# jzhangbs/MVSDF

Hardware: AMD Instinct MI355X
Metric: traced rays/sec (fwd+bwd, 10 sphere iters, 4 src views) (higher is better)
Workload: dtype f32x3

## Files before the change

include/mvsdf_hip.h:

```cpp
#ifndef MVSDF_HIP_H
#define MVSDF_HIP_H
#include <stddef.h>
#include <stdint.h>

#ifdef __cplusplus
extern "C" {
#endif

#define MVSDF_MAX_LAYERS 12

typedef struct {
    int n_layers;
    int K[MVSDF_MAX_LAYERS];
    int N[MVSDF_MAX_LAYERS];
    const float* wp[MVSDF_MAX_LAYERS];
    const float* bias[MVSDF_MAX_LAYERS];
    const float* w[MVSDF_MAX_LAYERS];
    int skip_layer;
    int multires;
    const void* wp16[MVSDF_MAX_LAYERS];
    int trace_dtype;
    unsigned skip_mask;
    const void* wx3[MVSDF_MAX_LAYERS];
} MvsdfNetDesc;

typedef struct {
    float r;
    float thr;
    float line_search_step;
    int line_step_iters;
    int st_iters;
    int n_steps;
    int n_secant;
    float dist_clip;
} MvsdfTraceParams;

enum {
    MVSDF_CNT_ROWS_SPHERE = 0,
    MVSDF_CNT_ROWS_SAMPLER = 1,
    MVSDF_CNT_ROWS_SECANT = 2,
    MVSDF_CNT_ROWS_MINSDF = 3,
    MVSDF_CNT_N_SECANT = 4,
    MVSDF_CNT_N_SAMPLER = 5,
    MVSDF_CNT_N_MINSDF = 6,
    MVSDF_CNT_N_SAMPLER_REST = 7,
    MVSDF_CNT_ROWS_SAMPLER_EVAL = 8,
    MVSDF_CNT_TAIL_NEXT = 9,
    MVSDF_CNT_TAIL_READY = 10,
    MVSDF_CNT_TAIL_WGS = 11,
    MVSDF_CNT_TAIL_ROWS = 12
};

int mvsdf_version(void);
int mvsdf_abi_struct_sizes(size_t* out);
const char* mvsdf_last_error(void);

size_t mvsdf_packed_floats(int N, int K);

int mvsdf_fold_pack(const float* v, const float* g, int N, int K, float* w, float* wp, float* wpT, void* stream);
int mvsdf_fold_pack_net(int n_layers, const float* const* v, const float* const* g, const int* N, const int* K, float* const* w,
                        float* const* wp, float* const* wpT, void* stream);
int mvsdf_fold_backward_net(int n_layers, const float* const* v, const float* const* g, const float* const* dW, const float* const* db,
                            const int* N, const int* K, float* const* dv, float* const* dg, float* const* dbias, int accumulate,
                            void* stream);
int mvsdf_fold_backward(const float* v, const float* g, const float* dW, int N, int K, float* dv, float* dg, void* stream);

size_t mvsdf_packed_bf16_bytes(int N, int K, int nsplit);
int mvsdf_pack_bf16w_net(int n_layers, const float* const* w, const int* N, const int* K, float* const* wp_rounded, void* stream);
int mvsdf_pack_bf16s_net(int n_layers, const float* const* w, const int* N, const int* K, void* const* wp16, void* stream);
int mvsdf_pack_bf16x3_net(int n_layers, const float* const* w, const int* N, const int* K, void* const* wp16, void* stream);
int mvsdf_pack_bf16x3t_net(int n_layers, const float* const* w, const int* N, const int* K, void* const* wx3t, void* stream);

int mvsdf_sdf_col0(const MvsdfNetDesc* net, const float* x, int n, float* y, int mt, void* stream);

int mvsdf_camera_rays(const float* uv, const float* pose, const float* intrinsics, int B, int P, float* ray_dirs, float* cam_loc,
                      void* stream);

int mvsdf_sphere_intersection(const float* cam_loc, const float* ray_dirs, int B, int P, float r, float* t, uint8_t* mask, void* stream);

size_t mvsdf_trace_workspace_bytes(int R);
size_t mvsdf_trace_workspace_bytes_n(int R, int n_steps);
int mvsdf_trace(const MvsdfNetDesc* net, const MvsdfTraceParams* tp, const float* cam_loc, const float* ray_dirs,
                const uint8_t* object_mask, int B, int P, int training, const float* intervals, const float* minsdf_steps,
                float* points, uint8_t* mask, float* dists, unsigned long long* counters, void* workspace,
                size_t workspace_bytes, int mt, int mt_samples, void* stream);
int mvsdf_trace_stage(int stage, const MvsdfNetDesc* net, const MvsdfTraceParams* tp, const float* cam_loc, const float* ray_dirs,
                      const uint8_t* object_mask, int B, int P, int training, const float* intervals, const float* minsdf_steps,
                      float* points, uint8_t* mask, float* dists, unsigned long long* counters, void* workspace,
                      size_t workspace_bytes, int mt, int mt_samples, void* stream);

size_t mvsdf_tracegen_state_bytes(int R);
int mvsdf_tracegen_init(const MvsdfTraceParams* tp, const float* cam_loc, const float* ray_dirs, const uint8_t* object_mask, int B, int P,
                        void* state, uint8_t* req, float* pts, unsigned long long* counters, void* stream);
int mvsdf_tracegen_step(const MvsdfTraceParams* tp, const float* cam_loc, const float* ray_dirs, int B, int P, void* state, const float* vals,
                        uint8_t* req, float* pts, unsigned long long* counters, void* stream);
int mvsdf_tracegen_finish(const MvsdfTraceParams* tp, const float* cam_loc, const float* ray_dirs, int B, int P, int training, const void* state,
                          float* points, uint8_t* mask, float* dists, unsigned long long* counters, void* workspace, size_t workspace_bytes,
                          void* stream);
int mvsdf_tracegen_rows(const MvsdfTraceParams* tp, int kind, const float* cam_loc, const float* ray_dirs, int B, int P, const float* zs, int n_list,
                        void* workspace, float* out_pts, void* stream);
int mvsdf_tracegen_reduce(const MvsdfTraceParams* tp, int kind, const float* cam_loc, const float* ray_dirs, int B, int P, int training,
                          const float* intervals, const float* minsdf_steps, const float* sv, float* points, uint8_t* mask, float* dists,
                          unsigned long long* counters, void* workspace, uint8_t* marks, void* stream);
int mvsdf_tracegen_secant(const MvsdfTraceParams* tp, int op, const float* cam_loc, const float* ray_dirs, int B, int P, int n_sec, const float* vals,
                          float* pts_out, float* points, float* dists, unsigned long long* counters, void* workspace, void* stream);

size_t mvsdf_sdf_ctx_floats(const MvsdfNetDesc* net, int M, int Mg);
int mvsdf_sdf_forward(const MvsdfNetDesc* net, const MvsdfNetDesc* netT, const float* x, int M, int Mg, float* y, float* nrm, float* ctx,
                      void* stream);
size_t mvsdf_sdf_bwd_ws_floats(const MvsdfNetDesc* net, int Mb);
int mvsdf_sdf_backward(const MvsdfNetDesc* net, const MvsdfNetDesc* netT, const float* x, int M, int Mg, int row0, int Mb, const float* dy,
                       const float* dn, const float* ctx, float* dW_cat, float* db_cat, float* dx, float* ws, void* stream);

int mvsdf_sdf_backward_pair(const MvsdfNetDesc* net, const MvsdfNetDesc* netT, int M, int Mg, int MbA, const float* dyA, const float* dnA, float* wsA,
                            int row0X, int MbX, const float* dyX, const float* dnX, float* wsX, float* dx, const float* ctx, void* stream);
int mvsdf_sdf_backward_finish(const MvsdfNetDesc* net, const MvsdfNetDesc* netT, int M, int Mg, int Mb, const float* dy, const float* ctx, float* ws,
                              int row0D, int MbD, const float* fbar, float* dW_cat, float* db_cat, void* stream);

size_t mvsdf_render_ctx_floats(const MvsdfNetDesc* net, int N);
size_t mvsdf_render_bwd_ws_floats(const MvsdfNetDesc* net, int N);
int mvsdf_render_forward(const MvsdfNetDesc* net, const float* points, const float* view, const float* normals, const float* feat,
                         int ldfeat, int N, int multires_view, float* rgb, float* ctx, void* stream);
int mvsdf_render_backward(const MvsdfNetDesc* net, const MvsdfNetDesc* netT, int N, int Nctx, const float* drgb, const float* ctx,
                          float* dW_cat, float* db_cat, float* din, float* ws, void* stream);

int mvsdf_feat_corr(const float* pts, int N, const int* view_start, int B, int V, int C, int H, int W, const float* feat,
                    const long long* feat_strides, const float* feat_src, const long long* src_strides, const float* cam,
                    const float* src_cams, const float* size, const float* center, float* loss_pp, float* dpts, void* stream);

int mvsdf_depth_carve(const float* pts, int pts_ld, int M, const float* depths, int B, int h, int w, const float* cams, const float* size,
                      const float* center, float out_thresh_perc, float far_thresh, float far_att, float near_thresh, float near_att, int use_invalid,
                      float* dist_r, float* weight, float* pts_world, void* stream);

int mvsdf_loss_terms(const float* rgb, const float* rgb_gt, const uint8_t* rgb_mask, int R, const float* grad_theta, int n_eik,
                     const float* eik_out, const float* dist_r, const float* dweight, int n_depth, const float* surf, int n_surf,
                     const long long* n_pos, const float* feat_pp, int n_feat, float w_rgb, float w_eik, float w_surf, float w_feat,
                     float w_depth, float smooth, int surf_on, int feat_on, const float* inv_counts, float* out, float* d_rgb, float* d_grad,
                     float* d_eik_out, float* d_surf, void* stream);

int mvsdf_partition_rays(const uint8_t* net_mask, const uint8_t* object_mask, const uint8_t* true_mask, const float* ray_dirs, int R,
                         long long* perm, long long* inv, long long* true_rows, long long* counts, float* view_sorted, void* stream);
int mvsdf_step_outputs(int R, int n_eik, int n_ds, int Nout, const long long* counts, const float* x_eval, const float* y_eval,
                       const float* n_eval, const long long* inv, const long long* true_rows, const float* rgb_sorted, int d_mask,
                       int e_mask, float* rgb_values, float* sdf_output, float* diff_pts, float* eik_out, float* points_hom, float* grad_theta,
                       float* surf, void* stream);
int mvsdf_step_backward_inputs(int stage, int n_eik, int n_ds, int N, int Nout, int n_true, const float* din, int din_ld, int din_feat0,
                               int din_nrm0, int use_geo, const float* d_diff, const float* dx, const float* view_sorted, const float* n_eval,
                               const long long* true_rows, const float* d_eo, const float* d_gth, const float* d_si, int d_mask, int e_mask,
                               float* dy, float* dn, void* stream);
int mvsdf_step_backward_fbar(int n_eik, int n_ds, int N, int Nout, const float* din, int din_ld, int use_geo, const float* d_diff, const float* dx,
                             const float* view_sorted, const float* n_eval, float* dy, float* fbar, void* stream);

int mvsdf_dsurf_select(const float* depths, const float* kinv, const float* einv, int N, int H, int W, const float* size, const float* center,
                       float bb, float jitter_rad, unsigned long long seed, int n, long long* idx, long long* counts, void* stream);
int mvsdf_dsurf_points(const float* depths, const float* kinv, const float* einv, int N, int H, int W, const float* size, const float* center,
                       float bb, float jitter_rad, unsigned long long seed, int n, const long long* idx_sorted, const long long* counts,
                       float* pts_on, float* pts_jit, void* stream);

size_t mvsdf_adam_ws_floats(void);
int mvsdf_adam_step(float* p, float* g, float* m, float* v, size_t n, float lr, double beta1, double beta2, float eps, int step, float max_norm,
                    float* norm_out, float* ws, void* stream);
int mvsdf_adam_step_scaled(float* p, float* g, float* m, float* v, size_t n, float lr, double beta1, double beta2, float eps, int step,
                           float max_norm, float grad_scale, float* norm_out, float* ws, void* stream);
int mvsdf_adam_step_fused(float* p, float* g, float* m, float* v, size_t n, float lr, double beta1, double beta2, float eps, int step,
                          float max_norm, float grad_scale, int zero_grad, float* norm_out, float* ws, void* stream);

int mvsdf_loss_prep(const uint8_t* net_mask, const uint8_t* obj_mask, const uint8_t* true_mask, int R, int B, uint8_t* hit, int* view_start,
                    long long* n_pos, void* stream);
int mvsdf_loss_scale(const float* const* g, float w_rgb, float w_eik, float w_surf, float w_feat, float w_depth, const float* d_rgb, float* g_rgb,
                     int n_rgb, const float* d_grad, float* g_grad, int n_grad, const float* d_eo, float* g_eo, int n_eo, const float* d_sf,
                     float* g_sf, int n_sf, float* coef_feat, void* stream);

int mvsdf_det_math(int op, const float* x, int n, float* y0, float* y1, void* stream);

#define MVSDF_STEP_MAX_LAYERS 24

typedef struct {
    int B, P;
    int n_eik;
    int n_ds;
    int n_sdf, n_render;
    int N[MVSDF_STEP_MAX_LAYERS];
    int K[MVSDF_STEP_MAX_LAYERS];
    unsigned skip_mask;
    int multires;
    int view_spec;
    int trace_dtype;
    int use_object_mask;
    MvsdfTraceParams tp;
    int mt, mt_samples;
} MvsdfStepDesc;

typedef struct {
    const float* v[MVSDF_STEP_MAX_LAYERS];
    const float* g[MVSDF_STEP_MAX_LAYERS];
    const float* b[MVSDF_STEP_MAX_LAYERS];
} MvsdfStepParams;

typedef struct {
    const float* uv; const float* pose; const float* intrinsics;
// ... 200 lines not shown
```

mvsdf_amd/_lib.py:

```python
import ctypes as C
import os

_HERE = os.path.dirname(os.path.abspath(__file__))
SO_PATH = os.environ.get('MVSDF_LIB') or os.path.join(_HERE, 'libmvsdf_hip.so')
MAX_LAYERS = 12
_lib = None


class NetDesc(C.Structure):
    _fields_ = [('n_layers', C.c_int), ('K', C.c_int * MAX_LAYERS), ('N', C.c_int * MAX_LAYERS),
                ('wp', C.c_void_p * MAX_LAYERS), ('bias', C.c_void_p * MAX_LAYERS), ('w', C.c_void_p * MAX_LAYERS),
                ('skip_layer', C.c_int), ('multires', C.c_int), ('wp16', C.c_void_p * MAX_LAYERS), ('trace_dtype', C.c_int), ('skip_mask', C.c_uint), ('wx3', C.c_void_p * MAX_LAYERS)]


class TraceParams(C.Structure):
    _fields_ = [('r', C.c_float), ('thr', C.c_float), ('line_search_step', C.c_float), ('line_step_iters', C.c_int),
                ('st_iters', C.c_int), ('n_steps', C.c_int), ('n_secant', C.c_int), ('dist_clip', C.c_float)]


class MvsdfError(RuntimeError):
    pass


def lib():
# ... 22 lines not shown
        L.mvsdf_adam_step_fused.argtypes = [C.c_void_p] * 4 + [C.c_size_t] + [C.c_float, C.c_double, C.c_double, C.c_float] + [C.c_int, C.c_float, C.c_float, C.c_int, C.c_void_p, C.c_void_p, C.c_void_p]
        L.mvsdf_loss_scale.argtypes = [C.c_void_p] + [C.c_float] * 5 + [C.c_void_p, C.c_void_p, C.c_int] * 4 + [C.c_void_p, C.c_void_p]
        i64, vp, f32 = C.c_int64, C.c_void_p, C.c_float
        L.mvsdf_mc_workspace_bytes.restype = C.c_size_t
        L.mvsdf_mc_workspace_bytes.argtypes = [i64] * 3
        L.mvsdf_mc_count.argtypes = [vp, vp, vp, f32, vp, C.c_size_t, vp]
        L.mvsdf_mc_emit.argtypes = [vp, vp, vp, f32, vp, vp, vp, C.c_size_t, vp, vp, vp, i64, i64, vp]
        L.mvsdf_mesh_cc_workspace_bytes.restype = C.c_size_t
        L.mvsdf_mesh_cc_workspace_bytes.argtypes = [i64, i64]
        L.mvsdf_mesh_components.argtypes = [vp, vp, i64, i64, vp, C.c_size_t, vp, vp, vp]
        L.mvsdf_mesh_select.argtypes = [vp, vp, i64, i64, C.c_int32] + [vp] * 5 + [C.c_size_t] + [vp] * 4 + [i64, i64, vp]
        L.mvsdf_smc_workspace_bytes.restype = C.c_size_t
        L.mvsdf_smc_workspace_bytes.argtypes = [i64, i64]
        L.mvsdf_smc_emit_workspace_bytes.restype = C.c_size_t
        L.mvsdf_smc_emit_workspace_bytes.argtypes = [i64, i64, i64]
        L.mvsdf_smc_coarse_points.argtypes = [vp, i64, i64, i64, i64, vp, vp]
        L.mvsdf_smc_seed.argtypes = [vp, i64, i64, f32, f32, vp, C.c_size_t, vp]
        L.mvsdf_smc_brick_points.argtypes = [vp, i64, i64, vp, C.c_size_t, i64, i64, vp, vp]
        L.mvsdf_smc_closure.argtypes = [vp, i64, i64, f32, i64, i64, vp, C.c_size_t, vp]
        L.mvsdf_smc_count.argtypes = [vp, i64, i64, f32, i64, vp, C.c_size_t, vp, C.c_size_t, vp]
        L.mvsdf_smc_emit.argtypes = [vp, i64, i64, f32, vp, vp, i64, vp, C.c_size_t, vp, C.c_size_t, vp, vp, vp, i64, i64, vp]
        L.mvsdf_mesh_cut_workspace_bytes.restype = C.c_size_t
        L.mvsdf_mesh_cut_workspace_bytes.argtypes = [i64, i64]
        L.mvsdf_mesh_cut.argtypes = [vp, vp, i64, i64, C.c_int32, C.c_int32, vp, C.c_size_t, vp, vp]
        L.mvsdf_mesh_trim.argtypes = [vp] * 4 + [i64, i64, vp, C.c_size_t] + [vp] * 4 + [i64, i64, vp]
        f64, u64, sz = C.c_double, C.c_uint64, C.c_size_t
        L.mvsdf_chamfer_key.restype = u64
        L.mvsdf_chamfer_key.argtypes = [u64, i64]
        for fn in ('mvsdf_chamfer_sample_workspace_bytes', 'mvsdf_chamfer_mask_workspace_bytes', 'mvsdf_chamfer_nearest_workspace_bytes'):
            getattr(L, fn).restype = sz
            getattr(L, fn).argtypes = [i64, i64]
        L.mvsdf_chamfer_downsample_workspace_bytes.restype = sz
        L.mvsdf_chamfer_downsample_workspace_bytes.argtypes = [i64]
        L.mvsdf_chamfer_sample_count.argtypes = [vp, vp, i64, i64, f64, i64, vp, sz, vp]
        L.mvsdf_chamfer_sample_emit.argtypes = [vp, vp, i64, i64, f64, vp, sz, vp, i64, vp]
        L.mvsdf_chamfer_downsample.argtypes = [vp, i64, f64, u64, i64, vp, sz, vp, vp]
        L.mvsdf_chamfer_mask.argtypes = [vp, vp, i64, vp, i64, vp, f64, vp, vp, vp, vp, sz, vp, vp, vp, vp]
        L.mvsdf_chamfer_nearest.argtypes = [vp, i64, vp, i64, f64, vp, sz, vp, vp]
        i32 = C.c_int32
        L.mvsdf_fusion_workspace_bytes.restype = sz
        L.mvsdf_fusion_workspace_bytes.argtypes = [i64] * 4
        L.mvsdf_fusion_fuse.argtypes = [vp, vp, vp, i64, i64, i64, vp, vp, vp, i32, i32, f64, f64, vp, sz, vp, vp, vp, vp]
        L.mvsdf_fusion_emit.argtypes = [vp, i64, i64, i64, i64, vp, sz, vp, vp, vp, vp, i64, vp]
        for fn in ('mvsdf_cloud_clean_workspace_bytes', 'mvsdf_cloud_compact_workspace_bytes'):
            getattr(L, fn).restype = sz
            getattr(L, fn).argtypes = [i64]
        L.mvsdf_cloud_knn.argtypes = [vp, i64, i32, vp, sz, vp, vp]
        L.mvsdf_cloud_components.argtypes = [vp, i64, f64, vp, sz, vp, vp]
        L.mvsdf_cloud_clean.argtypes = [vp, i64, i32, f64, f64, f64, vp, sz, vp, vp, vp, vp]
        L.mvsdf_cloud_compact.argtypes = [vp] * 5 + [i64, vp, sz] + [vp] * 4 + [i64, vp]
        L.mvsdf_raster_workspace_bytes.restype = sz
        L.mvsdf_raster_workspace_bytes.argtypes = [i64] * 5
        L.mvsdf_raster_draw.argtypes = [vp, vp, i64, i64, vp, i64, i64, i64, f64, i64, i32, vp, sz, vp]
        L.mvsdf_raster_resolve.argtypes = [i64, i64, i64, vp, sz, vp, vp, vp]
        L.mvsdf_raster_visibility.argtypes = [vp, i64, vp, i64, i64, i64, f64, vp, vp, f64, vp, sz, vp, vp]
        L.mvsdf_raster_colors.argtypes = [vp, vp, i64, vp, vp, i64, i64, i64, f64, vp, vp, vp, f64, f64, i32, f32, f32, f32, vp, sz, vp, vp, vp]
        for fn in ('mvsdf_featext_raw_floats', 'mvsdf_featext_pack_bytes', 'mvsdf_featext_workspace_bytes', 'mvsdf_featext_layer_workspace_bytes'):
            getattr(L, fn).restype = sz
        L.mvsdf_featext_raw_floats.argtypes = []
        L.mvsdf_featext_pack_bytes.argtypes = []
        L.mvsdf_featext_pack.argtypes = [vp, vp, sz, vp]
        L.mvsdf_featext_workspace_bytes.argtypes = [i64] * 3
        L.mvsdf_featext_forward.argtypes = [vp, vp, i64, i64, i64, vp, sz, vp, vp, vp, C.c_int, C.c_int, vp]
        L.mvsdf_featext_layer_workspace_bytes.argtypes = [C.c_int] * 5
        L.mvsdf_featext_layer.argtypes = [C.c_int, vp, vp, C.c_int, C.c_int, C.c_int, vp, C.c_int, vp, C.c_int, i64, i64, i64, vp, C.c_int, vp, sz, vp, vp]
        for fn in ('mvsdf_stereo_workspace_bytes', 'mvsdf_stereo_volume_offset'):
            getattr(L, fn).restype = sz
            getattr(L, fn).argtypes = [i64] * 4
        L.mvsdf_stereo_normalize.argtypes = [vp, i64, i64, vp, vp, vp]
        L.mvsdf_stereo_patches.argtypes = [vp, i64, i64, i64, i32, vp, vp]
        L.mvsdf_stereo_sweep.argtypes = [vp, i64, i64, i64, i64, i64] + [vp] * 7 + [sz] + [vp] * 5
        L.mvsdf_viewsel_bits_bytes.restype = sz
        L.mvsdf_viewsel_bits_bytes.argtypes = [i64, i64]
        L.mvsdf_viewsel_workspace_bytes.restype = sz
        L.mvsdf_viewsel_workspace_bytes.argtypes = [i64]
        L.mvsdf_viewsel_pack_dense.argtypes = [vp, i64, i64, vp, vp, vp]
        L.mvsdf_viewsel_pack_tracks.argtypes = [vp, vp, i64, i64, i64, vp, vp, vp]
        L.mvsdf_viewsel_scores.argtypes = [vp, vp, vp, i64, i64, f64, f64, f64, vp, sz, vp, vp, vp, vp]
        L.mvsdf_viewsel_depths.argtypes = [vp, vp, vp, i64, i64, i64, i64, vp, vp, vp]
        L.mvsdf_viewsel_weights_host.argtypes = [vp, vp, i64, f64, f64, f64, vp, vp]
        L.mvsdf_batch_args_bytes.restype = sz
        L.mvsdf_batch_args_bytes.argtypes = []
        L.mvsdf_batch_gather.argtypes = [vp, vp]
        for name in EXPORTS:
            getattr(L, name)
        _lib = L
    return _lib


EXPORTS = [
    'mvsdf_version', 'mvsdf_abi_struct_sizes', 'mvsdf_last_error', 'mvsdf_packed_floats', 'mvsdf_fold_pack', 'mvsdf_fold_backward', 'mvsdf_fold_pack_net', 'mvsdf_fold_backward_net', 'mvsdf_packed_bf16_bytes', 'mvsdf_pack_bf16w_net', 'mvsdf_pack_bf16s_net', 'mvsdf_pack_bf16x3_net', 'mvsdf_pack_bf16x3t_net',
    'mvsdf_sdf_col0', 'mvsdf_camera_rays', 'mvsdf_sphere_intersection', 'mvsdf_trace_workspace_bytes', 'mvsdf_trace_workspace_bytes_n', 'mvsdf_trace', 'mvsdf_trace_stage', 'mvsdf_det_math',
    'mvsdf_tracegen_state_bytes', 'mvsdf_tracegen_init', 'mvsdf_tracegen_step', 'mvsdf_tracegen_finish', 'mvsdf_tracegen_rows', 'mvsdf_tracegen_reduce',
    'mvsdf_tracegen_secant',
    'mvsdf_sdf_ctx_floats', 'mvsdf_sdf_forward', 'mvsdf_sdf_bwd_ws_floats', 'mvsdf_sdf_backward', 'mvsdf_sdf_backward_pair', 'mvsdf_sdf_backward_finish',
    'mvsdf_feat_corr', 'mvsdf_depth_carve', 'mvsdf_loss_terms', 'mvsdf_loss_prep', 'mvsdf_loss_scale', 'mvsdf_adam_ws_floats', 'mvsdf_adam_step', 'mvsdf_adam_step_scaled', 'mvsdf_adam_step_fused',
    'mvsdf_partition_rays', 'mvsdf_step_outputs', 'mvsdf_step_backward_inputs', 'mvsdf_step_backward_fbar', 'mvsdf_dsurf_select', 'mvsdf_dsurf_points',
    'mvsdf_render_ctx_floats', 'mvsdf_render_bwd_ws_floats', 'mvsdf_render_forward', 'mvsdf_render_backward',
    'mvsdf_step_create', 'mvsdf_step_destroy', 'mvsdf_step_forward', 'mvsdf_step_wait_counts', 'mvsdf_step_backward', 'mvsdf_step_set_timing', 'mvsdf_step_trace_times', 'mvsdf_step_times',
    'mvsdf_step_seq', 'mvsdf_step_counts_offset', 'mvsdf_step_wait_counts_seq', 'mvsdf_step_done_seq', 'mvsdf_step_can_defer', 'mvsdf_step_saved_offsets',
    'mvsdf_loss_layout', 'mvsdf_loss_forward', 'mvsdf_loss_backward',
    'mvsdf_mc_workspace_bytes', 'mvsdf_mc_count', 'mvsdf_mc_emit', 'mvsdf_mesh_cc_workspace_bytes', 'mvsdf_mesh_components', 'mvsdf_mesh_select',
    'mvsdf_smc_workspace_bytes', 'mvsdf_smc_emit_workspace_bytes', 'mvsdf_smc_coarse_points', 'mvsdf_smc_seed', 'mvsdf_smc_brick_points',
    'mvsdf_smc_closure', 'mvsdf_smc_count', 'mvsdf_smc_emit',
    'mvsdf_mesh_cut_workspace_bytes', 'mvsdf_mesh_cut', 'mvsdf_mesh_trim',
    'mvsdf_chamfer_key', 'mvsdf_chamfer_sample_workspace_bytes', 'mvsdf_chamfer_sample_count', 'mvsdf_chamfer_sample_emit',
    'mvsdf_chamfer_downsample_workspace_bytes', 'mvsdf_chamfer_downsample', 'mvsdf_chamfer_mask_workspace_bytes', 'mvsdf_chamfer_mask',
    'mvsdf_chamfer_nearest_workspace_bytes', 'mvsdf_chamfer_nearest',
    'mvsdf_fusion_workspace_bytes', 'mvsdf_fusion_fuse', 'mvsdf_fusion_emit',
    'mvsdf_cloud_clean_workspace_bytes', 'mvsdf_cloud_compact_workspace_bytes', 'mvsdf_cloud_knn', 'mvsdf_cloud_components', 'mvsdf_cloud_clean',
    'mvsdf_cloud_compact',
    'mvsdf_raster_workspace_bytes', 'mvsdf_raster_draw', 'mvsdf_raster_resolve', 'mvsdf_raster_visibility', 'mvsdf_raster_colors',
    'mvsdf_featext_raw_floats', 'mvsdf_featext_pack_bytes', 'mvsdf_featext_pack', 'mvsdf_featext_workspace_bytes', 'mvsdf_featext_forward',
    'mvsdf_featext_layer_workspace_bytes', 'mvsdf_featext_layer',
    'mvsdf_stereo_workspace_bytes', 'mvsdf_stereo_volume_offset', 'mvsdf_stereo_normalize', 'mvsdf_stereo_patches', 'mvsdf_stereo_sweep',
    'mvsdf_viewsel_bits_bytes', 'mvsdf_viewsel_workspace_bytes', 'mvsdf_viewsel_pack_dense', 'mvsdf_viewsel_pack_tracks', 'mvsdf_viewsel_scores',
    'mvsdf_viewsel_depths', 'mvsdf_viewsel_weights_host',
    'mvsdf_batch_args_bytes', 'mvsdf_batch_gather',
]


def check(rc, what=''):
    if rc != 0:
        raise MvsdfError('%s failed (code %d): %s' % (what or 'mvsdf call', rc, lib().mvsdf_last_error().decode()))


def ptr(t):
    if t is None:
        return None
    assert t.is_contiguous(), 'tensor must be contiguous'
    return C.c_void_p(t.data_ptr())


def stream_of(t):
    import torch
    if t.is_cuda:
        return C.c_void_p(torch.cuda.current_stream(t.device).cuda_stream)
    return C.c_void_p(0)
```

mvsdf_amd/csrc/basic.hip:

```cpp
#include <stdlib.h>
#include <string.h>
#include "tile_engine.h"
#include "trace_params.h"
#include "capi_util.h"
#include "det_math_pk.h"

__global__ __launch_bounds__(256) void k_fold(const float* __restrict__ v, const float* __restrict__ g, int N, int K, float* __restrict__ w) {
    const int j = blockIdx.x * 4 + (threadIdx.x >> 6), lane = threadIdx.x & 63;
    if (j >= N) return;
    const float* vr = v + (size_t)j * K;
    float ss = 0.0f;
    for (int k0 = 0; k0 < K; k0 += 64) {
        const float mine = (k0 + lane < K) ? vr[k0 + lane] : 0.0f;
        const int n = min(64, K - k0);
        for (int i = 0; i < n; ++i) {
            const float x = __int_as_float(__builtin_amdgcn_readlane(__float_as_int(mine), i));
            ss = fmaf(x, x, ss);
        }
    }
    const float a = g[j] / sqrtf(ss);
    for (int k = lane; k < K; k += 64) w[(size_t)j * K + k] = vr[k] * a;
}

__global__ void k_pack(const float* __restrict__ w, int N, int K, int transposed, float* __restrict__ wp) {
    const int No = transposed ? K : N, Ko = transposed ? N : K;
    const int KB = mv_kpad(Ko) / 16;
    const size_t total = (size_t)mv_ceil16(No) * mv_kpad(Ko);
    for (size_t idx = (size_t)blockIdx.x * blockDim.x + threadIdx.x; idx < total; idx += (size_t)gridDim.x * blockDim.x) {
        const int s = idx & 3, lane = (idx >> 2) & 63;
        const size_t blk = idx >> 8;
        const int kb = (int)(blk % KB), ct = (int)(blk / KB);
        const int o = ct * 16 + (lane & 15), i = kb * 16 + 4 * s + (lane >> 4);
        float val = 0.0f;
        if (o < No && i < Ko) val = transposed ? w[(size_t)i * K + o] : w[(size_t)o * K + i];
        wp[idx] = val;
    }
}

#define MV_FOLD_MAXL 24
struct FoldNetArgs {
    int n_layers;
    const float* v[MV_FOLD_MAXL]; const float* g[MV_FOLD_MAXL]; const float* dW[MV_FOLD_MAXL];
    float* w[MV_FOLD_MAXL]; float* wp[MV_FOLD_MAXL]; float* wpT[MV_FOLD_MAXL]; float* dv[MV_FOLD_MAXL]; float* dg[MV_FOLD_MAXL];
    const float* db[MV_FOLD_MAXL]; float* dbias[MV_FOLD_MAXL];
    int N[MV_FOLD_MAXL], K[MV_FOLD_MAXL];
    int accumulate;
};

__global__ __launch_bounds__(256) void k_fold_net(FoldNetArgs a) {
    const int l = blockIdx.y, N = a.N[l], K = a.K[l];
    const int j = blockIdx.x * 4 + (threadIdx.x >> 6), lane = threadIdx.x & 63;
    if (j >= N) return;
    const float* vr = a.v[l] + (size_t)j * K;
    if (!a.g[l]) {
        float* wr0 = a.w[l] + (size_t)j * K;
        for (int k = lane; k < K; k += 64) wr0[k] = vr[k];
        return;
    }
    float ss = 0.0f;
    for (int k0 = 0; k0 < K; k0 += 64) {
        const float mine = (k0 + lane < K) ? vr[k0 + lane] : 0.0f;
        const int n = min(64, K - k0);
        for (int i = 0; i < n; ++i) {
            const float x = __int_as_float(__builtin_amdgcn_readlane(__float_as_int(mine), i));
            ss = fmaf(x, x, ss);
        }
    }
    const float s = a.g[l][j] / sqrtf(ss);
    float* wr = a.w[l] + (size_t)j * K;
    for (int k = lane; k < K; k += 64) wr[k] = vr[k] * s;
}

__global__ void k_pack_net(FoldNetArgs a) {
    const int l = blockIdx.y >> 1, transposed = blockIdx.y & 1;
    float* wp = transposed ? a.wpT[l] : a.wp[l];
    if (!wp) return;
    const float* w = a.w[l];
    const int N = a.N[l], K = a.K[l];
    const int No = transposed ? K : N, Ko = transposed ? N : K;
    const int KB = mv_kpad(Ko) / 16;
    const size_t total = (size_t)mv_ceil16(No) * mv_kpad(Ko);
    for (size_t idx = (size_t)blockIdx.x * blockDim.x + threadIdx.x; idx < total; idx += (size_t)gridDim.x * blockDim.x) {
        const int s = idx & 3, lane = (idx >> 2) & 63;
        const size_t blk = idx >> 8;
        const int kb = (int)(blk % KB), ct = (int)(blk / KB);
        const int o = ct * 16 + (lane & 15), i = kb * 16 + 4 * s + (lane >> 4);
        float val = 0.0f;
        if (o < No && i < Ko) val = transposed ? w[(size_t)i * K + o] : w[(size_t)o * K + i];
        wp[idx] = val;
    }
}

__global__ void k_fold_bwd_net(FoldNetArgs a) {
    const int l = blockIdx.y, N = a.N[l], K = a.K[l];
    const int j = blockIdx.x * (blockDim.x >> 6) + (threadIdx.x >> 6), lane = threadIdx.x & 63;
    if (j >= N) return;
    const float* vr = a.v[l] + (size_t)j * K;
    const float* dr = a.dW[l] + (size_t)j * K;
    if (!a.g[l]) {
        float* dv0 = a.dv[l] + (size_t)j * K;
        for (int k = lane; k < K; k += 64) dv0[k] = a.accumulate ? dv0[k] + dr[k] : dr[k];
        if (lane == 0 && a.db[l]) a.dbias[l][j] = a.accumulate ? a.dbias[l][j] + a.db[l][j] : a.db[l][j];
        return;
    }
    float* dvr = a.dv[l] + (size_t)j * K;
    const bool acc = a.accumulate != 0;
    if (K <= 64 * 9) {
        float vv[9], dd[9], old[9];
        const float gj = a.g[l][j];
#pragma unroll
        for (int c = 0; c < 9; ++c) {
            const int k = 64 * c + lane, kc = k < K ? k : K - 1;
            const float x = vr[kc], y = dr[kc], z = acc ? dvr[kc] : 0.0f;
            vv[c] = k < K ? x : 0.0f; dd[c] = k < K ? y : 0.0f; old[c] = z;
        }
        float ss = 0.f, dot = 0.f;
#pragma unroll
        for (int c = 0; c < 9; ++c) if (64 * c < K) { ss = fmaf(vv[c], vv[c], ss); dot = fmaf(dd[c], vv[c], dot); }
        for (int o = 32; o > 0; o >>= 1) { ss += __shfl_xor(ss, o); dot += __shfl_xor(dot, o); }
        const float inv = 1.0f / sqrtf(ss);
        const float dgj = dot * inv, s = gj * inv;
#pragma unroll
        for (int c = 0; c < 9; ++c) {
            const int k = 64 * c + lane;
            if (k < K) { const float t = s * (dd[c] - dgj * vv[c] * inv); dvr[k] = acc ? old[c] + t : t; }
        }
        if (lane == 0) {
            a.dg[l][j] = acc ? a.dg[l][j] + dgj : dgj;
            if (a.db[l]) a.dbias[l][j] = acc ? a.dbias[l][j] + a.db[l][j] : a.db[l][j];
        }
        return;
    }
    float ss = 0.f, dot = 0.f;
    for (int k = lane; k < K; k += 64) { ss = fmaf(vr[k], vr[k], ss); dot = fmaf(dr[k], vr[k], dot); }
    for (int o = 32; o > 0; o >>= 1) { ss += __shfl_xor(ss, o); dot += __shfl_xor(dot, o); }
    const float inv = 1.0f / sqrtf(ss);
    const float dgj = dot * inv, s = a.g[l][j] * inv;
    for (int k = lane; k < K; k += 64) {
        const float t = s * (dr[k] - dgj * vr[k] * inv);
        dvr[k] = acc ? dvr[k] + t : t;
    }
    if (lane == 0) {
        a.dg[l][j] = acc ? a.dg[l][j] + dgj : dgj;
        if (a.db[l]) a.dbias[l][j] = acc ? a.dbias[l][j] + a.db[l][j] : a.db[l][j];
    }
}

__global__ void k_fold_bwd(const float* __restrict__ v, const float* __restrict__ g, const float* __restrict__ dW, int N, int K,
                           float* __restrict__ dv, float* __restrict__ dg) {
    const int j = blockIdx.x * (blockDim.x >> 6) + (threadIdx.x >> 6), lane = threadIdx.x & 63;
    if (j >= N) return;
    const float* vr = v + (size_t)j * K;
    const float* dr = dW + (size_t)j * K;
    float ss = 0.f, dot = 0.f;
    for (int k = lane; k < K; k += 64) { ss = fmaf(vr[k], vr[k], ss); dot = fmaf(dr[k], vr[k], dot); }
    for (int o = 32; o > 0; o >>= 1) { ss += __shfl_xor(ss, o); dot += __shfl_xor(dot, o); }
    const float nrm = sqrtf(ss), inv = 1.0f / nrm;
    const float dgj = dot * inv;
    const float a = g[j] * inv;
    for (int k = lane; k < K; k += 64) dv[(size_t)j * K + k] = a * (dr[k] - dgj * vr[k] * inv);
    if (lane == 0) dg[j] = dgj;
}

__global__ void k_camera_rays(const float* __restrict__ uv, const float* __restrict__ pose, const float* __restrict__ Kin, int B, int P,
                              float* __restrict__ dirs, float* __restrict__ cam_loc) {
    const int idx = blockIdx.x * blockDim.x + threadIdx.x;
    if (idx >= B * P) return;
    const int b = idx / P;
    const float* p = pose + 16 * b;
    const float* k = Kin + 16 * b;
    const float fx = k[0], fy = k[5], cx = k[2], cy = k[6], sk = k[1];
    const float cl[3] = {p[3], p[7], p[11]};
    if (idx == b * P) { cam_loc[3 * b] = cl[0]; cam_loc[3 * b + 1] = cl[1]; cam_loc[3 * b + 2] = cl[2]; }
    const float x = uv[2 * (size_t)idx] + 0.5f, y = uv[2 * (size_t)idx + 1] + 0.5f, z = 1.0f;
    const float xl = (x - cx + cy * sk / fy - sk * y / fy) / fx * z;
    const float yl = (y - cy) / fy * z;
    const float h[4] = {xl, yl, z, 1.0f};
    float wv[3];
    for (int r = 0; r < 3; ++r) {
        float acc = 0.0f;
        for (int c = 0; c < 4; ++c) acc = fmaf(p[4 * r + c], h[c], acc);
        wv[r] = acc - cl[r];
    }
    float nn = sqrtf(wv[0] * wv[0] + wv[1] * wv[1] + wv[2] * wv[2]);
    if (nn < 1e-12f) nn = 1e-12f;
    dirs[3 * (size_t)idx] = wv[0] / nn;
    dirs[3 * (size_t)idx + 1] = wv[1] / nn;
    dirs[3 * (size_t)idx + 2] = wv[2] / nn;
}

__global__ void k_sphere_intersection(const float* __restrict__ cam_loc, const float* __restrict__ dirs, int B, int P, float r,
                                      float* __restrict__ t, uint8_t* __restrict__ mask) {
    const int idx = blockIdx.x * blockDim.x + threadIdx.x;
    if (idx >= B * P) return;
    const float* c = cam_loc + 3 * (idx / P);
    const float* d = dirs + 3 * (size_t)idx;
    const float dot = fmaf(d[2], c[2], fmaf(d[1], c[1], d[0] * c[0]));
    const float nrm = sqrtf(c[0] * c[0] + c[1] * c[1] + c[2] * c[2]);
    const float under = dot * dot - (nrm * nrm - r * r);
    const bool hit = under > 0.0f;
    float a = 0.0f, b = 0.0f;
    if (hit) { const float s = sqrtf(under); a = s * -1.0f - dot; b = s * 1.0f - dot; }
    t[2 * (size_t)idx] = a < 0.0f ? 0.0f : a;
    t[2 * (size_t)idx + 1] = b < 0.0f ? 0.0f : b;
    mask[idx] = hit ? 1 : 0;
}

template <int MT, int NTW, int NW, bool XR = false>
__global__ __launch_bounds__(64 * NW) void k_sdf_col0(MvNet net, const float* __restrict__ x, int n, float* __restrict__ y) {
    extern __shared__ __attribute__((aligned(16))) float smem[];
    constexpr int ROWS = 16 * MT;
    const int tid = threadIdx.x, d0 = 3 + 6 * net.multires;
    float* act = smem;
    float* pe = act + ROWS * net.S;
    float* pts = pe + ((ROWS * d0 + 3) & ~3);
    float* out = pts + ROWS * 4;
    const int row0 = blockIdx.x * ROWS;
    for (int i = tid; i < ROWS * 3; i += 64 * NW) {
        const int row = row0 + i / 3;
        pts[i] = row < n ? x[3 * (size_t)row0 + i] : 0.0f;
    }
    __syncthreads();
    mv_sdf_eval_col0<MT, NTW, NW, XR>(net, act, pe, pts, out, tid);
    if (tid < ROWS && row0 + tid < n) y[row0 + tid] = out[tid];
}

struct PackBfArgs { const float* w[MV_MAXL]; uint16_t* wp[MV_MAXL]; int N[MV_MAXL], K[MV_MAXL], nsplit[MV_MAXL]; int tr; };
__global__ void k_pack_bf16_net(PackBfArgs a) {
// ... 107 lines not shown
    y0[i] = a;
    if (y1) y1[i] = b;
}

template <int MT, int NTW, int NW, bool XR = false>
static int launch_col0(const MvNet& net, const float* x, int n, float* y, hipStream_t s) {
    const int rows = 16 * MT, d0 = 3 + 6 * net.multires;
    const size_t lds = ((size_t)rows * net.S + ((rows * d0 + 3) & ~3) + rows * 4 + rows) * 4;
    hipError_t e = hipFuncSetAttribute((const void*)k_sdf_col0<MT, NTW, NW, XR>, hipFuncAttributeMaxDynamicSharedMemorySize, (int)lds);
    if (e != hipSuccess) return mv_check(e, "mvsdf_sdf_col0: LDS attribute");
    hipLaunchKernelGGL((k_sdf_col0<MT, NTW, NW, XR>), dim3((n + rows - 1) / rows), dim3(64 * NW), lds, s, net, x, n, y);
    return mv_check(hipGetLastError(), "mvsdf_sdf_col0");
}

extern "C" {

int mvsdf_version(void) { return 100; }

size_t mvsdf_packed_floats(int N, int K) { return mv_packed_floats(N, K); }

int mvsdf_fold_pack(const float* v, const float* g, int N, int K, float* w, float* wp, float* wpT, void* stream) {
    if (!v || !g || N <= 0 || K <= 0 || !w) return mv_fail(-1, "mvsdf_fold_pack: bad arguments (w must be given)");
    hipStream_t s = (hipStream_t)stream;
    hipLaunchKernelGGL(k_fold, dim3((N + 3) / 4), dim3(256), 0, s, v, g, N, K, w);
    const size_t total = mv_packed_floats(N, K);
    const int blocks = (int)((total + 255) / 256 < 1024 ? (total + 255) / 256 : 1024);
    if (wp) hipLaunchKernelGGL(k_pack, dim3(blocks), dim3(256), 0, s, w, N, K, 0, wp);
    if (wpT) hipLaunchKernelGGL(k_pack, dim3(blocks), dim3(256), 0, s, w, N, K, 1, wpT);
    return mv_check(hipGetLastError(), "mvsdf_fold_pack");
}

static int fill_fold_args(FoldNetArgs& a, int n_layers, const int* N, const int* K, int* maxN, size_t* maxTot) {
    if (n_layers < 1 || n_layers > MV_FOLD_MAXL || !N || !K) return mv_fail(-1, "fold (net): bad layer count / dims");
    memset(&a, 0, sizeof(a));
    a.n_layers = n_layers;
    *maxN = 0; *maxTot = 0;
    for (int l = 0; l < n_layers; ++l) {
        if (N[l] <= 0 || K[l] <= 0) return mv_fail(-1, "fold (net): bad dims");
        a.N[l] = N[l]; a.K[l] = K[l];
        if (N[l] > *maxN) *maxN = N[l];
        const size_t t = mv_packed_floats(N[l], K[l]) > mv_packed_floats(K[l], N[l]) ? mv_packed_floats(N[l], K[l]) : mv_packed_floats(K[l], N[l]);
        if (t > *maxTot) *maxTot = t;
    }
    return 0;
}

int mvsdf_fold_pack_net(int n_layers, const float* const* v, const float* const* g, const int* N, const int* K, float* const* w,
                        float* const* wp, float* const* wpT, void* stream) {
    FoldNetArgs a;
    int maxN; size_t maxTot;
    int rc = fill_fold_args(a, n_layers, N, K, &maxN, &maxTot);
    if (rc) return rc;
    if (!v || !g || !w || !wp || !wpT) return mv_fail(-1, "mvsdf_fold_pack_net: null argument");
    for (int l = 0; l < n_layers; ++l) {
        if (!v[l] || !w[l]) return mv_fail(-1, "mvsdf_fold_pack_net: null layer pointer");
        a.v[l] = v[l]; a.g[l] = g[l]; a.w[l] = w[l]; a.wp[l] = wp[l]; a.wpT[l] = wpT[l];
    }
    hipStream_t s = (hipStream_t)stream;
    hipLaunchKernelGGL(k_fold_net, dim3((maxN + 3) / 4, n_layers), dim3(256), 0, s, a);
    const int blocks = (int)((maxTot + 255) / 256 < 256 ? (maxTot + 255) / 256 : 256);
    hipLaunchKernelGGL(k_pack_net, dim3(blocks, 2 * n_layers), dim3(256), 0, s, a);
    return mv_check(hipGetLastError(), "mvsdf_fold_pack_net");
}

int mvsdf_fold_backward_net(int n_layers, const float* const* v, const float* const* g, const float* const* dW, const float* const* db,
                            const int* N, const int* K, float* const* dv, float* const* dg, float* const* dbias, int accumulate,
                            void* stream) {
    FoldNetArgs a;
    int maxN; size_t maxTot;
    int rc = fill_fold_args(a, n_layers, N, K, &maxN, &maxTot);
    if (rc) return rc;
    if (!v || !g || !dW || !dv || !dg || ((db == nullptr) != (dbias == nullptr))) return mv_fail(-1, "mvsdf_fold_backward_net: null argument");
    a.accumulate = accumulate;
    for (int l = 0; l < n_layers; ++l) {
        if (!v[l] || !dW[l] || !dv[l] || (g[l] && !dg[l])) return mv_fail(-1, "mvsdf_fold_backward_net: null layer pointer");
        a.v[l] = v[l]; a.g[l] = g[l]; a.dW[l] = dW[l]; a.dv[l] = dv[l]; a.dg[l] = dg[l];
        if (db) {
            if ((db[l] == nullptr) != (dbias[l] == nullptr)) return mv_fail(-1, "mvsdf_fold_backward_net: db / dbias must pair up");
            a.db[l] = db[l]; a.dbias[l] = dbias[l];
        }
    }
    hipLaunchKernelGGL(k_fold_bwd_net, dim3((maxN + 3) / 4, n_layers), dim3(256), 0, (hipStream_t)stream, a);
    return mv_check(hipGetLastError(), "mvsdf_fold_backward_net");
}

int mvsdf_fold_backward(const float* v, const float* g, const float* dW, int N, int K, float* dv, float* dg, void* stream) {
    if (!v || !g || !dW || !dv || !dg || N <= 0 || K <= 0) return mv_fail(-1, "mvsdf_fold_backward: bad arguments");
    hipLaunchKernelGGL(k_fold_bwd, dim3((N + 3) / 4), dim3(256), 0, (hipStream_t)stream, v, g, dW, N, K, dv, dg);
    return mv_check(hipGetLastError(), "mvsdf_fold_backward");
}

int mvsdf_camera_rays(const float* uv, const float* pose, const float* intrinsics, int B, int P, float* ray_dirs, float* cam_loc,
                      void* stream) {
    if (!uv || !pose || !intrinsics || !ray_dirs || !cam_loc || B <= 0 || P <= 0) return mv_fail(-1, "mvsdf_camera_rays: bad arguments");
    hipLaunchKernelGGL(k_camera_rays, dim3((B * P + 255) / 256), dim3(256), 0, (hipStream_t)stream, uv, pose, intrinsics, B, P, ray_dirs,
                       cam_loc);
    return mv_check(hipGetLastError(), "mvsdf_camera_rays");
}

int mvsdf_sphere_intersection(const float* cam_loc, const float* ray_dirs, int B, int P, float r, float* t, uint8_t* mask, void* stream) {
    if (!cam_loc || !ray_dirs || !t || !mask || B <= 0 || P <= 0) return mv_fail(-1, "mvsdf_sphere_intersection: bad arguments");
    hipLaunchKernelGGL(k_sphere_intersection, dim3((B * P + 255) / 256), dim3(256), 0, (hipStream_t)stream, cam_loc, ray_dirs, B, P, r, t, mask);
    return mv_check(hipGetLastError(), "mvsdf_sphere_intersection");
}

size_t mvsdf_packed_bf16_bytes(int N, int K, int nsplit) { return mv_packed_bf16_elems(N, K, nsplit) * 2; }

int mvsdf_pack_bf16s_net(int n_layers, const float* const* w, const int* N, const int* K, void* const* wp16, void* stream) {
    if (n_layers < 1 || n_layers > MV_MAXL || !w || !N || !K || !wp16) return mv_fail(-1, "mvsdf_pack_bf16s_net: bad arguments");
    PackBfArgs a;
    memset(&a, 0, sizeof(a));
    size_t maxTot = 0;
    for (int l = 0; l < n_layers; ++l) {
        if (!w[l] || !wp16[l] || N[l] <= 0 || K[l] <= 0) return mv_fail(-1, "mvsdf_pack_bf16s_net: null layer pointer / bad dims");
        a.w[l] = w[l]; a.wp[l] = (uint16_t*)wp16[l]; a.N[l] = N[l]; a.K[l] = K[l]; a.nsplit[l] = 0;
        const size_t t = mv_packed_bf16_elems(N[l], K[l], 0);
        if (t > maxTot) maxTot = t;
    }
    const int blocks = (int)((maxTot + 255) / 256 < 256 ? (maxTot + 255) / 256 : 256);
    hipLaunchKernelGGL(k_pack_bf16_net, dim3(blocks, n_layers), dim3(256), 0, (hipStream_t)stream, a);
    return mv_check(hipGetLastError(), "mvsdf_pack_bf16s_net");
}

static int pack_x3_net(int n_layers, const float* const* w, const int* N, const int* K, void* const* out, int tr, void* stream) {
    if (n_layers < 1 || n_layers > MV_MAXL || !w || !N || !K || !out) return mv_fail(-1, "mvsdf_pack_bf16x3_net / mvsdf_pack_bf16x3t_net: bad arguments");
    PackBfArgs a;
    memset(&a, 0, sizeof(a));
    a.tr = tr;
    size_t maxTot = 0;
    for (int l = 0; l < n_layers; ++l) {
        if (!w[l] || !out[l] || N[l] <= 0 || K[l] <= 0) return mv_fail(-1, "mvsdf_pack_bf16x3_net / mvsdf_pack_bf16x3t_net: null layer pointer / bad dims");
        a.w[l] = w[l]; a.wp[l] = (uint16_t*)out[l]; a.N[l] = N[l]; a.K[l] = K[l]; a.nsplit[l] = 0;
        const size_t t = 3 * (tr ? mv_packed_bf16_elems(K[l], N[l], 0) : mv_packed_bf16_elems(N[l], K[l], 0));
        if (t > maxTot) maxTot = t;
    }
    const int blocks = (int)((maxTot + 255) / 256 < 512 ? (maxTot + 255) / 256 : 512);
    hipLaunchKernelGGL(k_pack_bf16x3_net, dim3(blocks, n_layers), dim3(256), 0, (hipStream_t)stream, a);
    return mv_check(hipGetLastError(), "mvsdf_pack_bf16x3_net");
}
int mvsdf_pack_bf16x3_net(int n_layers, const float* const* w, const int* N, const int* K, void* const* wp16, void* stream) {
    return pack_x3_net(n_layers, w, N, K, wp16, 0, stream);
}
int mvsdf_pack_bf16x3t_net(int n_layers, const float* const* w, const int* N, const int* K, void* const* wx3t, void* stream) {
    return pack_x3_net(n_layers, w, N, K, wx3t, 1, stream);
}

int mvsdf_pack_bf16w_net(int n_layers, const float* const* w, const int* N, const int* K, float* const* wp_rounded, void* stream) {
    if (n_layers < 1 || n_layers > MV_MAXL || !w || !N || !K || !wp_rounded) return mv_fail(-1, "mvsdf_pack_bf16w_net: bad arguments");
    PackBfArgs a;
    memset(&a, 0, sizeof(a));
    size_t maxTot = 0;
    for (int l = 0; l < n_layers; ++l) {
        if (!w[l] || !wp_rounded[l] || N[l] <= 0 || K[l] <= 0) return mv_fail(-1, "mvsdf_pack_bf16w_net: null layer pointer / bad dims");
        a.w[l] = w[l]; a.wp[l] = (uint16_t*)wp_rounded[l]; a.N[l] = N[l]; a.K[l] = K[l];
        const size_t t = mv_packed_floats(N[l], K[l]);
        if (t > maxTot) maxTot = t;
    }
    const int blocks = (int)((maxTot + 255) / 256 < 256 ? (maxTot + 255) / 256 : 256);
    hipLaunchKernelGGL(k_pack_round_net, dim3(blocks, n_layers), dim3(256), 0, (hipStream_t)stream, a);
    return mv_check(hipGetLastError(), "mvsdf_pack_bf16w_net");
}

int mvsdf_sdf_col0(const MvsdfNetDesc* desc, const float* x, int n, float* y, int mt, void* stream) {
    if (!x || !y || n <= 0) return mv_fail(-1, "mvsdf_sdf_col0: bad arguments");
    hipStream_t s = (hipStream_t)stream;
    if (desc && desc->trace_dtype == 1) return mv_fail(-2, "mvsdf_sdf_col0: trace_dtype 1 (bf16 weights AND 8-bit activations) was removed in round 5: use 3 (bf16x2: same speed, parity-checked)");
// ... 275 lines not shown
```

mvsdf_amd/csrc/diff_mlp.hip:

```cpp
#include <stdlib.h>
#include "layer_kernels.h"
#include "chain_x3.h"
#include "capi_util.h"
#include "step_internal.h"

__global__ void k_pe_global(const float* __restrict__ x, int M, int multires, float* __restrict__ H0, int ld) {
    const int T = 3 * multires + 1;
    const int idx = blockIdx.x * blockDim.x + threadIdx.x;
    if (idx >= M * T) return;
    const int row = idx / T, j = idx - row * T, d0 = 3 + 6 * multires;
    const float* xr = x + (size_t)row * 3;
    float* h = H0 + (size_t)row * ld;
    if (j < 3 * multires) {
        const int m = j / 3, c = j - 3 * m;
        float s, co;
        dm_sincos(xr[c] * (float)(1 << m), &s, &co);
        h[3 + 6 * m + c] = s;
        h[6 + 6 * m + c] = co;
    } else {
        for (int c = 0; c < 3; ++c) h[c] = xr[c];
        for (int c = d0; c < ld; ++c) h[c] = 0.0f;
    }
}

// ... 102 lines not shown
    static int v = -1;
    if (v < 0) { const char* e = mv_dev_env("MVSDF_CHAIN_W8"); v = e ? atoi(e) : 0; }
    return v != 0;
}

static int stride_for(const MvNet& a, const MvNet& b) { return a.S > b.S ? a.S : b.S; }

struct SdfLayout {
    int nl, d0, ld0;
    size_t H0, A[MV_MAXL], Z[MV_MAXL], U[MV_MAXL], Sg[MV_MAXL], E, G0, total;
};
static SdfLayout sdf_ctx_layout(const MvNet& net, int M, int Mg) {
    SdfLayout o;
    memset(&o, 0, sizeof(o));
    o.nl = net.n_layers; o.d0 = 3 + 6 * net.multires; o.ld0 = (o.d0 + 3) & ~3;
    size_t p = 0;
    o.H0 = p; p += (size_t)M * o.ld0;
    for (int l = 1; l < o.nl; ++l) { o.A[l] = p; p += (size_t)M * net.L[l].K; }
    for (int l = 0; l < o.nl - 1; ++l) { o.Z[l] = p; p += (size_t)M * net.L[l].N; }
    for (int l = 1; l < o.nl - 1; ++l) { o.U[l] = p; p += (size_t)Mg * net.L[l - 1].N; }
    for (int l = 0; l < o.nl - 1; ++l) { o.Sg[l] = p; p += (size_t)Mg * net.L[l].N; }
    o.E = p; p += (size_t)Mg * o.ld0;
    o.G0 = p; p += (size_t)Mg * o.ld0;
    o.total = p;
    return o;
}
struct SdfBwdLayout {
    size_t VB[MV_MAXL], ZB2[MV_MAXL], ZB[MV_MAXL], HB[2], H0B, slabA, slabB, bslab, total;
    int nchunks, chunk;
    size_t maxnk;
};
static size_t wgrad_net_slab_floats(const MvNet& net, int nchunks) {
    size_t t = 0;
    for (int l = 0; l < net.n_layers; ++l) t += (size_t)nchunks * net.L[l].N * net.L[l].K;
    return t;
}
static size_t wgrad_net_bslab_floats(const MvNet& net, int nchunks) {
    size_t t = 0;
    for (int l = 0; l < net.n_layers; ++l) t += (size_t)nchunks * net.L[l].N;
    return t;
}
static SdfBwdLayout sdf_bwd_layout(const MvNet& net, int Mb) {
    SdfBwdLayout o;
    memset(&o, 0, sizeof(o));
    const int nl = net.n_layers, ld0 = ((3 + 6 * net.multires) + 3) & ~3;
    size_t p = 0;
    int maxw = 0;
    for (int l = 0; l < nl; ++l) { maxw = net.L[l].K > maxw ? net.L[l].K : maxw; maxw = net.L[l].N > maxw ? net.L[l].N : maxw; }
    for (int l = 0; l < nl; ++l) { o.VB[l] = p; p += (size_t)Mb * (l == 0 ? ld0 : net.L[l].K); }
    for (int l = 0; l < nl - 1; ++l) { o.ZB2[l] = p; p += (size_t)Mb * net.L[l].N; }
    for (int l = 0; l < nl - 1; ++l) { o.ZB[l] = p; p += (size_t)Mb * net.L[l].N; }
    o.HB[0] = p; p += (size_t)Mb * maxw;
    o.HB[1] = p; p += (size_t)Mb * maxw;
    o.H0B = p; p += (size_t)Mb * ld0;
    o.chunk = MV_WG_CHUNK;
    o.nchunks = (Mb + o.chunk - 1) / o.chunk;
    if (o.nchunks < 1) o.nchunks = 1;
    o.maxnk = 0;
    for (int l = 0; l < nl; ++l) { const size_t nk = (size_t)net.L[l].N * net.L[l].K; o.maxnk = nk > o.maxnk ? nk : o.maxnk; }
    o.slabA = p; p += wgrad_net_slab_floats(net, o.nchunks);
    o.slabB = p; p += (size_t)o.nchunks * maxw;
    o.bslab = p; p += wgrad_net_bslab_floats(net, o.nchunks);
    o.total = p;
    return o;
}

static void wgrad_net_layers(WgradNetArgs& a, int l0, int n, int M, int nchunks, float* slab, float* bslab, float* dW_cat, float* db_cat) {
    size_t so = 0, bo = 0, wo = 0, b2 = 0;
    for (int l = l0; l < l0 + n; ++l) {
        WgradLayer& L = a.L[l];
        L.M = M; L.nchunks = nchunks; L.ch0 = 0; L.nch = nchunks;
        L.nbx = (L.Ki + 63) / 64; L.nby = (L.No + 63) / 64;
        L.slab = slab + so; so += (size_t)nchunks * L.No * L.Ki;
        L.bslab = bslab + bo; bo += (size_t)nchunks * L.No;
        L.dW = dW_cat + wo; wo += (size_t)L.No * L.Ki;
        L.db = db_cat + b2; b2 += L.No;
    }
}
static hipError_t wgrad_launch(WgradNetArgs& a, hipStream_t s) {
    int blk = 0;
    for (int l = 0; l < a.n_layers; ++l) {
        WgradLayer& L = a.L[l];
        L.blk0 = blk; blk += L.nbx * L.nby * L.nch;
    }
    if (a.colX) { a.col_blk0 = blk; blk += ((a.col_n + 63) / 64) * a.col_nch; }
    static int xcd_env = -2;
    if (xcd_env == -2) { const char* e = mv_dev_env("MVSDF_WG_XCD"); xcd_env = (e && *e) ? atoi(e) : -1; }
    a.nblocks = blk;
    a.xcd_runs = xcd_env >= 0 ? (xcd_env != 0) : 1;
    const int grid = a.xcd_runs ? ((blk + 127) / 128) * 128 : blk;
    if (blk > 0) hipLaunchKernelGGL(k_wgrad_net, dim3(grid), dim3(MV_THREADS), 0, s, a);
    return hipGetLastError();
}
static hipError_t wgrad_reduce(WgradNetArgs& a, hipStream_t s) {
    size_t wo = 0, b2 = 0;
    for (int l = 0; l < a.n_layers; ++l) {
        WgradLayer& L = a.L[l];
        L.woff = (unsigned)wo; wo += (size_t)L.No * L.Ki;
        L.boff = (unsigned)b2; b2 += L.No;
    }
    if (wo + b2 >= 0xffffffffull) return hipErrorInvalidValue;
    a.wtotal = (unsigned)wo; a.btotal = (unsigned)b2;
    const unsigned total = a.wtotal + a.btotal;
    const int blocks = (int)((total + 255) / 256 > 4096 ? 4096 : (total + 255) / 256);
    hipLaunchKernelGGL(k_reduce_net, dim3(blocks), dim3(256), 0, s, a);
    return hipGetLastError();
}
static hipError_t launch_wgrad_net(WgradNetArgs& a, hipStream_t s) {
    hipError_t e = wgrad_launch(a, s);
    return e != hipSuccess ? e : wgrad_reduce(a, s);
}
static void wgrad_colsum(WgradNetArgs& a, const float* X, int ld, int M, int n, int layer, int nchunks, float* colslab) {
    a.colX = X; a.col_ld = ld; a.col_M = M; a.col_n = n; a.col_layer = layer; a.col_nchunks = nchunks; a.col_ch0 = 0; a.col_nch = nchunks; a.colslab = colslab;
}

static int mv_single_skip(const MvNet& net) {
    const unsigned m = net.skip_mask;
    if (!m) return -1;
    if (m & (m - 1)) return -2;
    return __builtin_ctz(m);
}

static int mv_chain_mt(int tiles16) {
    static const int env = [] { const char* e = mv_dev_env("MVSDF_CHAIN_MT"); return e ? atoi(e) : 0; }();
    if (env == 1 || env == 2) return env;
    const int rounds1 = (tiles16 + 255) / 256, rounds2 = (tiles16 + 511) / 512;
    return 1.76 * rounds2 < rounds1 ? 2 : 1;
}
int mv_chain_split_pays(const MvsdfNetDesc* d, int E, int M) {
    MvNet net;
    if (E < 16 || E >= M || mv_make_net(d, &net) || mv_chain_ntw(net) != 2 || mv_chain_w8()) return 0;
    auto cost = [](int tiles16) { const int r1 = (tiles16 + 255) / 256, r2 = (tiles16 + 511) / 512; return 1.76 * r2 < r1 ? 1.76 * r2 : 1.0 * r1; };
    return cost((M - E + 15) / 16) < cost((M + 15) / 16) ? 1 : 0;
}

static bool mv_chain_x3_on() {
    static const int env = [] {
        const char* e = mv_dev_env("MVSDF_CHAIN_X3");
        const char* f = mv_dev_env("MVSDF_FUSE");
        if ((f && atoi(f) == 0) || mv_dev_env("MVSDF_SPLIT_CHAINS") || mv_dev_env("MVSDF_CHAIN_W8")) return 0;
        return e ? atoi(e) : 1;
    }();
    return env != 0;
}
int mv_chain_x3_enabled() { return mv_chain_x3_on() ? 1 : 0; }
static int mv_x3_nets(const MvsdfNetDesc* d, const MvsdfNetDesc* dT, bool needT, MvNetBf* xn, MvNetBf* xnT) {
    if (!mv_chain_x3_on() || mv_make_net_x3(d, xn)) return 1;
    if (needT) { if (!dT || mv_make_net_x3(dT, xnT)) return 1; }
    else *xnT = *xn;
    xnT->skip_mask = xn->skip_mask; xnT->multires = xn->multires;
    const int S16 = xn->S > xnT->S ? xn->S : xnT->S;
    xn->S = xnT->S = S16;
    return 0;
}
static int mv_chain_mt_x3(int tiles16) {
    static const int env = [] { const char* e = mv_dev_env("MVSDF_CHAIN_MT"); return e ? atoi(e) : 0; }();
    if (env == 1 || env == 2) return env;
    const int rounds1 = (tiles16 + 255) / 256, rounds2 = (tiles16 + 511) / 512;
    return 1.45 * rounds2 < rounds1 ? 2 : 1;
}

#ifndef MV_X3_PD1
#define MV_X3_PD1 4
#endif
#ifndef MV_X3_PD2
#define MV_X3_PD2 0
// ... 472 lines not shown
    return v;
}
int mv_delta_is_chain() { return mv_delta_chain(); }

static int sdf_delta_pass(const MvNet& net, const MvNet& netT, const SdfLayout& lo, const SdfBwdLayout& bl, const float* ctx, float* ws, int row0D,
                          int MbD, const float* fbar, hipStream_t s) {
    if (!mv_delta_chain()) {
        DeltaArgs d;
        memset(&d, 0, sizeof(d));
        d.nl1 = lo.nl - 1; d.rows = MbD; d.fbar = fbar;
        for (int l = 0; l < lo.nl - 1; ++l) {
            d.N[l] = net.L[l].N;
            d.Sg[l] = ctx + lo.Sg[l] + (size_t)row0D * net.L[l].N;
            d.ZB[l] = ws + bl.ZB[l] + (size_t)row0D * net.L[l].N;
        }
        hipLaunchKernelGGL(k_delta_apply<false>, dim3(MbD, lo.nl - 1), dim3(256), 0, s, d);
        return mv_check(hipGetLastError(), "sdf_delta_pass");
    }
    const int ntw_b = mv_chain_ntw(net);
    const int nl = lo.nl, S = stride_for(net, netT);
    ChainArgs c;
    memset(&c, 0, sizeof(c));
    const size_t r0 = (size_t)row0D;
    c.net = net; c.netT = netT; c.S = S; c.M = MbD; c.row_ld0 = lo.ld0;
    c.ld_dy = net.L[nl - 1].N; c.dy_col0 = fbar; c.accum = 1;
    for (int l = 0; l < nl - 1; ++l) { c.Z[l] = ctx + lo.Z[l] + r0 * net.L[l].N; c.ZB[l] = ws + bl.ZB[l] + r0 * net.L[l].N; }
    const bool w8w = mv_chain_w8();
    const int mt = (ntw_b == 2 && !w8w) ? mv_chain_mt((MbD + 15) / 16) : 1;
    const size_t lds = (size_t)16 * mt * (S + lo.d0) * sizeof(float);
    const dim3 grid((MbD + 16 * mt - 1) / (16 * mt));
    if (mt == 2) {
        { static size_t hw = 0; MV_TRY(mv_lds_limit(k_chain_bwd<2, 1, 16>, lds, hw)); }
        hipLaunchKernelGGL((k_chain_bwd<2, 1, 16>), grid, dim3(1024), lds, s, c);
    }
    else if (ntw_b == 2 && !w8w) hipLaunchKernelGGL((k_chain_bwd<1, 1, 16>), grid, dim3(1024), lds, s, c);
    else if (ntw_b == 2) hipLaunchKernelGGL((k_chain_bwd<1, 2, 8>), grid, dim3(512), lds, s, c);
    else if (!w8w) hipLaunchKernelGGL((k_chain_bwd<1, 2, 16>), grid, dim3(1024), lds, s, c);
    else hipLaunchKernelGGL((k_chain_bwd<1, 4, 8>), grid, dim3(512), lds, s, c);
    return mv_check(hipGetLastError(), "sdf_delta_pass");
}

static void sdf_wgrad_operands(WgradNetArgs& wa, int l0, const MvNet& net, const SdfLayout& lo, const SdfBwdLayout& bl, const float* dy, const float* ctx,
                               float* ws) {
    const int nl = lo.nl;
    for (int l = 0; l < nl; ++l) {
        WgradLayer& L = wa.L[l0 + l];
        const bool last = (l == nl - 1);
        L.No = net.L[l].N; L.Ki = net.L[l].K;
        L.P1 = last ? dy : ws + bl.ZB[l]; L.ldp1 = L.No;
        L.Q1 = l == 0 ? ctx + lo.H0 : ctx + lo.A[l]; L.ldq1 = l == 0 ? lo.ld0 : net.L[l].K;
        if (!last) { L.P2 = ctx + lo.Sg[l]; L.ldp2 = L.No; L.Q2 = ws + bl.VB[l]; L.ldq2 = L.ldq1; }
    }
}

extern "C" {

int mvsdf_sdf_backward_finish(const MvsdfNetDesc* d, const MvsdfNetDesc* dT, int M, int Mg, int Mb, const float* dy, const float* ctx, float* ws,
                              int row0D, int MbD, const float* fbar, float* dW_cat, float* db_cat, void* stream) {
    MvNet net, netT;
    int rc = mv_make_net(d, &net);
    if (rc) return rc;
    rc = mv_make_net_mode(dT, &netT, 2);
    if (rc) return rc;
    if (!dy || !ctx || !ws || !dW_cat || !db_cat || Mb <= 0 || Mb > Mg || Mg > M || MbD < 0 || row0D < 0 || row0D + MbD > Mb || (MbD > 0 && !fbar))
        return mv_fail(-1, "mvsdf_sdf_backward_finish: bad arguments");
    if (!mv_chain_ntw(net)) return mv_fail(-3, "mvsdf_sdf_backward_finish: network too wide for the fused chain kernels");
    hipStream_t s = (hipStream_t)stream;
    const SdfLayout lo = sdf_ctx_layout(net, M, Mg);
    const SdfBwdLayout bl = sdf_bwd_layout(net, Mb);
    const int nl = lo.nl;
    if (MbD > 0) {
        rc = sdf_delta_pass(net, netT, lo, bl, ctx, ws, row0D, MbD, fbar, s);
        if (rc) return rc;
    }
    WgradNetArgs wa;
    memset(&wa, 0, sizeof(wa));
    wa.n_layers = nl; wa.chunk = bl.chunk;
    sdf_wgrad_operands(wa, 0, net, lo, bl, dy, ctx, ws);
    wgrad_net_layers(wa, 0, nl, Mb, bl.nchunks, ws + bl.slabA, ws + bl.bslab, dW_cat, db_cat);
    const int Ki = net.L[nl - 1].K;
    wgrad_colsum(wa, ws + bl.VB[nl - 1], Ki, Mb, Ki, nl - 1, bl.nchunks, ws + bl.slabB);
    MV_TRY(launch_wgrad_net(wa, s));
    return mv_check(hipGetLastError(), "mvsdf_sdf_backward_finish");
}

}

struct RenderLayout { size_t A[MV_MAXL], rgb, total; };
static RenderLayout render_layout(const MvNet& net, int N) {
    RenderLayout o;
    memset(&o, 0, sizeof(o));
    size_t p = 0;
    for (int l = 0; l < net.n_layers; ++l) { o.A[l] = p; p += (size_t)N * net.L[l].K; }
    o.rgb = p; p += (size_t)N * net.L[net.n_layers - 1].N;
    o.total = p;
    return o;
}
struct RenderBwdLayout { size_t ZB[MV_MAXL], slab, bslab, total; int chunk, nchunks; };
static RenderBwdLayout render_bwd_layout(const MvNet& net, int N) {
    RenderBwdLayout o;
    memset(&o, 0, sizeof(o));
    size_t p = 0, maxnk = 0;
    int maxw = 0;
    for (int l = 0; l < net.n_layers; ++l) {
        o.ZB[l] = p; p += (size_t)N * net.L[l].N;
        const size_t nk = (size_t)net.L[l].N * net.L[l].K;
        maxnk = nk > maxnk ? nk : maxnk;
        maxw = net.L[l].N > maxw ? net.L[l].N : maxw;
    }
    o.chunk = MV_WG_CHUNK; o.nchunks = (N + MV_WG_CHUNK - 1) / MV_WG_CHUNK; if (o.nchunks < 1) o.nchunks = 1;
    o.slab = p; p += wgrad_net_slab_floats(net, o.nchunks);
    o.bslab = p; p += wgrad_net_bslab_floats(net, o.nchunks);
    o.total = p;
    return o;
}

__global__ void k_render_input(const float* __restrict__ points, const float* __restrict__ view, const float* __restrict__ normals,
                               const float* __restrict__ feat, int ldfeat, int N, int mv, int K0, float* __restrict__ A0) {
    const size_t idx = (size_t)blockIdx.x * blockDim.x + threadIdx.x;
    if (idx >= (size_t)N * K0) return;
    const int row = (int)(idx / K0), k = (int)(idx - (size_t)row * K0);
    const float v = mv_render_input_raw(points, view, normals, feat, ldfeat, mv, row, k);
    A0[idx] = v;
}

extern "C" {

size_t mvsdf_render_ctx_floats(const MvsdfNetDesc* d, int N) {
    MvNet net;
    if (mv_make_net_mode(d, &net, 1)) return 0;
    return render_layout(net, N).total;
}
size_t mvsdf_render_bwd_ws_floats(const MvsdfNetDesc* d, int N) {
    MvNet net;
    if (mv_make_net_mode(d, &net, 1)) return 0;
    return render_bwd_layout(net, N).total;
}

int mvsdf_render_forward(const MvsdfNetDesc* d, const float* points, const float* view, const float* normals, const float* feat,
                         int ldfeat, int N, int multires_view, float* rgb, float* ctx, void* stream) {
    MvNet net;
    int rc = mv_make_net_mode(d, &net, 1);
    if (rc) return rc;
    if (!points || !view || !normals || !feat || !rgb || !ctx || N <= 0) return mv_fail(-1, "mvsdf_render_forward: bad arguments");
    const int nl = net.n_layers, K0 = net.L[0].K;
    if ((multires_view & ~0x3ff) || (multires_view & 0xff) > 16 || (multires_view & 0x300) == 0x300)
        return mv_fail(-1, "mvsdf_render_forward: bad multires_view / mode bits");
    if (K0 <= 3 + mv_render_dv(multires_view) + mv_render_dn(multires_view))
        return mv_fail(-1, "mvsdf_render_forward: first layer too narrow for cat[points, PE(view), normals, feat]");
    hipStream_t s = (hipStream_t)stream;
    const RenderLayout lo = render_layout(net, N);
    static int fuse_r = -1;
    if (fuse_r < 0) { const char* e = mv_dev_env("MVSDF_FUSE"); fuse_r = e ? atoi(e) : 1; }
    const int ntw_r = mv_chain_ntw(net);
    if (fuse_r && ntw_r && net.L[nl - 1].NT <= 2) {
        RenderChainArgs c;
        memset(&c, 0, sizeof(c));
        c.net = net; c.S = net.S; c.N = N; c.mv = multires_view; c.K0 = K0;
        c.points = points; c.view = view; c.normals = normals; c.feat = feat; c.ldfeat = ldfeat;
        for (int l = 0; l < nl; ++l) c.A[l] = ctx + lo.A[l];
        c.rgb_ctx = ctx + lo.rgb; c.rgb = rgb;
        constexpr int MTC = 1, NWC = 8;
        const bool w8 = mv_chain_w8();
        const dim3 grid((N + 16 * MTC - 1) / (16 * MTC));
        const size_t ldsr = (size_t)16 * MTC * net.S * sizeof(float);
        if (ntw_r == 2 && !w8) hipLaunchKernelGGL((k_render_chain_fwd<MTC, 1, 16>), grid, dim3(1024), ldsr, s, c);
// ... 65 lines not shown
static void render_wgrad_operands(WgradNetArgs& wa, int l0, const MvNet& net, const RenderLayout& lo, const RenderBwdLayout& bl, const float* ctx, float* ws) {
    for (int l = 0; l < net.n_layers; ++l) {
        WgradLayer& L = wa.L[l0 + l];
        L.No = net.L[l].N; L.Ki = net.L[l].K;
        L.P1 = ws + bl.ZB[l]; L.ldp1 = L.No;
        L.Q1 = ctx + lo.A[l]; L.ldq1 = L.Ki;
    }
}

extern "C" {

int mvsdf_render_backward(const MvsdfNetDesc* d, const MvsdfNetDesc* dT, int N, int Nctx, const float* drgb, const float* ctx, float* dW_cat,
                          float* db_cat, float* din, float* ws, void* stream) {
    MvNet net, netT;
    int rc = mv_make_net_mode(d, &net, 1);
    if (rc) return rc;
    rc = mv_make_net_mode(dT, &netT, 2);
    if (rc) return rc;
    if (!drgb || !ctx || !dW_cat || !db_cat || !din || !ws || N <= 0 || Nctx < N) return mv_fail(-1, "mvsdf_render_backward: bad arguments");
    hipStream_t s = (hipStream_t)stream;
    rc = render_backward_chain(net, netT, N, Nctx, drgb, ctx, din, ws, s);
    if (rc) return rc;
    const RenderLayout lo = render_layout(net, Nctx);
    const RenderBwdLayout bl = render_bwd_layout(net, N);
    WgradNetArgs wa;
    memset(&wa, 0, sizeof(wa));
    wa.n_layers = net.n_layers; wa.chunk = bl.chunk;
    render_wgrad_operands(wa, 0, net, lo, bl, ctx, ws);
    wgrad_net_layers(wa, 0, net.n_layers, N, bl.nchunks, ws + bl.slab, ws + bl.bslab, dW_cat, db_cat);
    MV_TRY(launch_wgrad_net(wa, s));
    return mv_check(hipGetLastError(), "mvsdf_render_backward");
}

}

int mv_render_backward_chain(const MvsdfNetDesc* d, const MvsdfNetDesc* dT, int N, int Nctx, const float* drgb, const long long* drgb_rows, const float* ctx,
                             float* din, float* ws, const long long* cnt, void* stream) {
    MvNet net, netT;
    int rc = mv_make_net_mode(d, &net, 1);
    if (rc) return rc;
    rc = mv_make_net_mode(dT, &netT, 2);
    if (rc) return rc;
    if (!drgb || !ctx || !din || !ws || N <= 0 || Nctx < N) return mv_fail(-1, "mv_render_backward_chain: bad arguments");
    rc = render_backward_chain(net, netT, N, Nctx, drgb, ctx, din, ws, (hipStream_t)stream, drgb_rows, cnt);
    return rc ? rc : mv_check(hipGetLastError(), "mv_render_backward_chain");
}

int mv_sdf_backward_delta(const MvsdfNetDesc* d, const MvsdfNetDesc* dT, int M, int Mg, int Mb, const float* ctx, float* ws, int row0D, int MbD,
                          const float* fbar, void* stream) {
    MvNet net, netT;
    int rc = mv_make_net(d, &net);
    if (rc) return rc;
    rc = mv_make_net_mode(dT, &netT, 2);
    if (rc) return rc;
    if (!ctx || !ws || !fbar || Mb <= 0 || Mb > Mg || Mg > M || MbD <= 0 || row0D < 0 || row0D + MbD > Mb) return mv_fail(-1, "mv_sdf_backward_delta: bad arguments");
    if (!mv_chain_ntw(net)) return mv_fail(-3, "mv_sdf_backward_delta: network too wide for the fused chain kernels");
    return sdf_delta_pass(net, netT, sdf_ctx_layout(net, M, Mg), sdf_bwd_layout(net, Mb), ctx, ws, row0D, MbD, fbar, (hipStream_t)stream);
}

int mv_sdf_backward_delta_fbar(const MvsdfNetDesc* d, int M, int Mg, int Mb, const float* ctx, float* ws, int row0D, int MbD, int Nout, const float* din,
                               int din_ld, int use_geo, const float* d_diff, const float* dx, const float* view_sorted, const float* n_eval, float* dy,
                               float* fbar, const long long* cnt, void* stream) {
    MvNet net;
    int rc = mv_make_net(d, &net);
    if (rc) return rc;
    if (!ctx || !ws || !fbar || !view_sorted || !n_eval || !dy || Mb <= 0 || Mb > Mg || Mg > M || MbD <= 0 || row0D < 0 || row0D + MbD > Mb)
        return mv_fail(-1, "mv_sdf_backward_delta_fbar: bad arguments");
    const SdfLayout lo = sdf_ctx_layout(net, M, Mg);
    const SdfBwdLayout bl = sdf_bwd_layout(net, Mb);
    DeltaArgs a;
    memset(&a, 0, sizeof(a));
    a.nl1 = lo.nl - 1; a.rows = MbD;
    for (int l = 0; l < lo.nl - 1; ++l) {
        a.N[l] = net.L[l].N;
        a.Sg[l] = ctx + lo.Sg[l] + (size_t)row0D * net.L[l].N;
        a.ZB[l] = ws + bl.ZB[l] + (size_t)row0D * net.L[l].N;
    }
    a.d_diff = d_diff; a.din = din; a.dx = dx; a.view_sorted = view_sorted; a.n_hit = n_eval + 3 * (size_t)row0D;
    a.din_ld = din_ld; a.use_geo = use_geo; a.Nout = Nout; a.dy_hit = dy + (size_t)row0D * Nout; a.fbar_out = fbar; a.cnt = cnt;
    hipLaunchKernelGGL(k_delta_apply<true>, dim3(MbD), dim3(256), 0, (hipStream_t)stream, a);
    return mv_check(hipGetLastError(), "mv_sdf_backward_delta_fbar");
}

int mv_step_wgrad(const MvsdfNetDesc* sd, const MvsdfNetDesc* rd, int M, int Mg, int Mb, const float* dy, const float* ctx, float* wsA, int N, int Nctx,
                  const float* rctx, float* rws, float* dW_s, float* db_s, float* dW_r, float* db_r, const long long* cnt, int cnt_base, void* stream) {
    MvNet net, rnet;
    int rc = mv_make_net(sd, &net);
    if (rc) return rc;
    const bool with_r = N > 0 && rctx && rws;
    if (with_r) { rc = mv_make_net_mode(rd, &rnet, 1); if (rc) return rc; }
    if (!dy || !ctx || !wsA || !dW_s || !db_s || Mb <= 0 || Mb > Mg || Mg > M || (with_r && (!dW_r || !db_r || Nctx < N)))
        return mv_fail(-1, "mv_step_wgrad: bad arguments");
    const SdfLayout lo = sdf_ctx_layout(net, M, Mg);
    const SdfBwdLayout bl = sdf_bwd_layout(net, Mb);
    const int nl = lo.nl, nr = with_r ? rnet.n_layers : 0;
    if (nl + nr > MV_WG_MAXL) return mv_fail(-1, "mv_step_wgrad: too many layers");
    WgradNetArgs wa;
    memset(&wa, 0, sizeof(wa));
    wa.n_layers = nl + nr; wa.chunk = bl.chunk;
    sdf_wgrad_operands(wa, 0, net, lo, bl, dy, ctx, wsA);
    wgrad_net_layers(wa, 0, nl, Mb, bl.nchunks, wsA + bl.slabA, wsA + bl.bslab, dW_s, db_s);
    if (with_r) {
        const RenderLayout rlo = render_layout(rnet, Nctx);
        const RenderBwdLayout rbl = render_bwd_layout(rnet, N);
        if (rbl.chunk != bl.chunk) return mv_fail(-1, "mv_step_wgrad: chunk sizes differ");
        render_wgrad_operands(wa, nl, rnet, rlo, rbl, rctx, rws);
        wgrad_net_layers(wa, nl, nr, N, rbl.nchunks, rws + rbl.slab, rws + rbl.bslab, dW_r, db_r);
    }
    const int Ki = net.L[nl - 1].K;
    wgrad_colsum(wa, wsA + bl.VB[nl - 1], Ki, Mb, Ki, nl - 1, bl.nchunks, wsA + bl.slabB);
    if (cnt) {
        wa.cnt = cnt; wa.col_mbase = cnt_base;
        for (int l = 0; l < nl; ++l) wa.L[l].mbase = cnt_base;
        for (int l = nl; l < nl + nr; ++l) wa.L[l].mbase = 0;
    }
    MV_TRY(launch_wgrad_net(wa, (hipStream_t)stream));
    return mv_check(hipGetLastError(), "mv_step_wgrad");
}

int mv_step_can_defer(const MvsdfNetDesc* sdf, const MvsdfNetDesc* sdfT, const MvsdfNetDesc* rnd, const MvsdfNetDesc* rndT) {
    MvNet net, netT, rnet, rnetT;
    if (mv_make_net(sdf, &net) || mv_make_net_mode(sdfT, &netT, 2) || mv_make_net_mode(rnd, &rnet, 1) || mv_make_net_mode(rndT, &rnetT, 2)) return 0;
    if (!mv_chain_ntw(net) || mv_delta_chain()) return 0;
    const char* e = mv_dev_env("MVSDF_FUSE");
    if (e && atoi(e) == 0) return 0;
    const int ntw_rb = mv_chain_ntw(rnet);
    if (!ntw_rb) return 0;
    for (int l = 1; l < rnet.n_layers; ++l) if (rnetT.L[l].NT > 8 * ntw_rb) return 0;
    return net.n_layers + rnet.n_layers <= MV_WG_MAXL ? 1 : 0;
}

#ifdef MV_CHAIN_PROBE
extern "C" int mv_chain_probe_read(unsigned long long* out, int reset) {
    if (hipMemcpyFromSymbol(out, HIP_SYMBOL(g_chain_ph), sizeof(unsigned long long) * 256) != hipSuccess) return -1;
    if (reset) { static unsigned long long z[256]; if (hipMemcpyToSymbol(HIP_SYMBOL(g_chain_ph), z, sizeof z) != hipSuccess) return -1; }
    return 0;
}
#endif
```

mvsdf_amd/csrc/layer_kernels.h:

```cpp
#pragma once
#include "tile_engine.h"
#include "step_internal.h"

enum {
    PRO_PLAIN = 0,
    PRO_SIG_MUL,
    PRO_SIG_BCAST,
    PRO_ZBAR,
    PRO_TANH_BWD
};
enum {
    EPI_SOFTPLUS = 0,
    EPI_BIAS,
    EPI_SPLIT,
    EPI_SBAR,
    EPI_RELU,
    EPI_TANH,
    EPI_RELU_MASK
};

struct LayerArgs {
    MvLayer L;
    int S;
    int M, Mg;
// ... 67 lines not shown
        const float sig = in.z;
        const float u = in.u;
        float ub = sig * acc;
        if (a.skip_next) ub = dm_div_sqrt2(ub);
        a.out0[(size_t)row * a.ld0 + col] = ub;
        a.out1[(size_t)row * a.ld1 + col] = u * acc * dm_sigmoid_prime100(sig);
    } else if (EPI == EPI_RELU) {
        a.out0[(size_t)row * a.ld0 + col] = fmaxf(acc + a.L.bias[col], 0.0f);
    } else if (EPI == EPI_TANH) {
        a.out0[(size_t)row * a.ld0 + col] = tanhf(acc + a.L.bias[col]);
    } else if (EPI == EPI_RELU_MASK) {
        a.out0[(size_t)row * a.ld0 + col] = in.add > 0.0f ? acc : 0.0f;
    }
}

template <int PRO, int EPI, int MT, int NTW>
__global__ __launch_bounds__(MV_THREADS) void k_layer(LayerArgs a) {
    extern __shared__ __attribute__((aligned(16))) float smem[];
    constexpr int ROWS = 16 * MT;
    const int tid = threadIdx.x, lane = tid & 63, w = __builtin_amdgcn_readfirstlane(tid >> 6), r = lane & 15, q = lane >> 4;
    const int row0 = blockIdx.x * ROWS, S = a.S, K = a.L.K, Kp = a.L.KB * 16, N = a.L.N;
    float* act = smem;
    for (int base = 0; base < ROWS * Kp; base += MV_THREADS * 8) {
        float v[8];
#pragma unroll
        for (int u = 0; u < 8; ++u) {
            const int idx = base + u * MV_THREADS + tid;
            const int rr = idx / Kp, k = idx - rr * Kp, row = row0 + rr;
            v[u] = 0.0f;
            if (idx < ROWS * Kp && row < a.M && k < K) v[u] = mv_prologue<PRO>(a, row, k);
        }
#pragma unroll
        for (int u = 0; u < 8; ++u) {
            const int idx = base + u * MV_THREADS + tid;
            const int rr = idx / Kp, k = idx - rr * Kp;
            if (idx < ROWS * Kp) act[rr * S + mv_perm(k)] = v[u];
        }
    }
    __syncthreads();
    const int NT = a.L.NT;
    const int per = (NT + 3) >> 2;
    for (int g0 = 0; g0 < per; g0 += NTW) {
        const int ct0 = w * per + g0;
        int ntw = min(per - g0, NT - ct0);
        ntw = ntw < 0 ? 0 : (ntw > NTW ? NTW : ntw);
        f32x4 acc[MT][NTW];
        mv_zero_acc<MT, NTW>(acc);
        if (ntw > 0) mv_gemm_dispatch<MT, NTW>(a.L, act, S, ct0, ntw, acc, lane);
#pragma unroll
        for (int t = 0; t < NTW; ++t) {
            if (t < ntw) {
                const int col = (ct0 + t) * 16 + r;
                if (col < N) {
                    EpiIn in[MT][4];
#pragma unroll
                    for (int m = 0; m < MT; ++m)
#pragma unroll
                        for (int i = 0; i < 4; ++i) {
                            const int row = row0 + m * 16 + 4 * q + i;
                            in[m][i] = EpiIn{0.f, 0.f, 0.f};
                            if (row < a.M) in[m][i] = mv_epilogue_load<EPI>(a, row, col);
                        }
#pragma unroll
                    for (int m = 0; m < MT; ++m)
#pragma unroll
                        for (int i = 0; i < 4; ++i) {
                            const int row = row0 + m * 16 + 4 * q + i;
                            if (row < a.M) mv_epilogue<EPI>(a, row, col, acc[m][t][i], in[m][i]);
                        }
                }
            }
        }
    }
    if (EPI == EPI_SOFTPLUS || EPI == EPI_SBAR) {
        if (EPI == EPI_SOFTPLUS && a.skip_next) {
            for (int idx = tid; idx < ROWS * a.d0; idx += MV_THREADS) {
                const int rr = idx / a.d0, j = idx - rr * a.d0, row = row0 + rr;
                if (row < a.M) a.out0[(size_t)row * a.ld0 + N + j] = dm_div_sqrt2(a.pe[(size_t)row * a.ldpe + j]);
            }
        }
    }
}

__device__ __forceinline__ void wg_stage(const float* __restrict__ src, int ld, int row_lo, int row_hi, int c0, int ncols, float* __restrict__ dst,
                                         int LD, int tid) {
    const bool vec = ((ld & 3) == 0) && ((c0 & 3) == 0) && ((((size_t)src) & 15) == 0);
    if (vec) {
        float4 v[4];
#pragma unroll
        for (int u = 0; u < 4; ++u) {
            const int idx = u * MV_THREADS + tid, rr = idx >> 4, c4 = (idx & 15) * 4, row = row_lo + rr;
            v[u] = make_float4(0.f, 0.f, 0.f, 0.f);
            if (row < row_hi) {
                if (c0 + c4 + 3 < ncols) v[u] = *(const float4*)(src + (size_t)row * ld + c0 + c4);
                else {
                    float t[4] = {0.f, 0.f, 0.f, 0.f};
                    for (int e = 0; e < 4; ++e) if (c0 + c4 + e < ncols) t[e] = src[(size_t)row * ld + c0 + c4 + e];
                    v[u] = make_float4(t[0], t[1], t[2], t[3]);
                }
            }
        }
#pragma unroll
        for (int u = 0; u < 4; ++u) {
            const int idx = u * MV_THREADS + tid, rr = idx >> 4, c4 = (idx & 15) * 4;
            *(float4*)(dst + rr * LD + c4) = v[u];
        }
    } else {
        float v[16];
#pragma unroll
        for (int u = 0; u < 16; ++u) {
            const int idx = u * MV_THREADS + tid, rr = idx >> 6, c = idx & 63, row = row_lo + rr;
            v[u] = (row < row_hi && c0 + c < ncols) ? src[(size_t)row * ld + c0 + c] : 0.0f;
        }
#pragma unroll
        for (int u = 0; u < 16; ++u) {
            const int idx = u * MV_THREADS + tid, rr = idx >> 6, c = idx & 63;
            dst[rr * LD + c] = v[u];
        }
    }
}

#ifdef MV_CHAIN_PROBE
__device__ unsigned long long g_chain_ph[16][16];
#define CH_PH_DECL unsigned long long chp_[16] = {0, 0, 0, 0, 0, 0, 0, 0, 0, 0, 0, 0, 0, 0, 0, 0}; unsigned long long cht_ = wall_clock64();
#define CH_PH(i) { const unsigned long long t_ = wall_clock64(); chp_[i] += t_ - cht_; cht_ = t_; }
#define CH_PH_END if (blockIdx.x == 0 && (threadIdx.x & 63) == 0) { for (int i_ = 0; i_ < 16; ++i_) atomicAdd(&g_chain_ph[threadIdx.x >> 6][i_], chp_[i_]); }
#define WG_PH_END(blk) if ((int)blockIdx.x == (blk) && (threadIdx.x & 63) == 0) { for (int i_ = 0; i_ < 16; ++i_) atomicAdd(&g_chain_ph[8 + (threadIdx.x >> 6)][i_], chp_[i_]); }
#else
#define CH_PH_DECL
#define CH_PH(i)
#define CH_PH_END
#define WG_PH_END(blk)
#endif

#define MV_WG_MAXL 16
#define MV_WG_CHUNK 256
struct WgradLayer {
    const float* P1; const float* Q1; const float* P2; const float* Q2;
    int ldp1, ldq1, ldp2, ldq2;
    int No, Ki, nbx, nby;
    int M;
    int mbase;
    int nchunks;
    int ch0, nch;
    int blk0;
    float* slab; float* bslab;
    float* dW; float* db;
    unsigned woff, boff;
};
struct WgradNetArgs {
    int n_layers, chunk;
    WgradLayer L[MV_WG_MAXL];
    const float* colX; int col_ld, col_M, col_n, col_layer, col_nchunks, col_ch0, col_nch, col_blk0;
    float* colslab;
    unsigned wtotal, btotal;
    const long long* cnt; int col_mbase;
    int xcd_runs, nblocks;
};

__device__ __forceinline__ int mv_wg_rows(const WgradNetArgs& a, const WgradLayer& L) { return a.cnt ? L.mbase + (int)a.cnt[0] : L.M; }
__device__ __forceinline__ int mv_wg_col_rows(const WgradNetArgs& a) { return a.cnt ? a.col_mbase + (int)a.cnt[0] : a.col_M; }

__device__ __forceinline__ void mv_colsum_block(const WgradNetArgs& a, int local, float* scratch) {
    float (*red)[64] = (float (*)[64])scratch;
    const int nbx = (a.col_n + 63) / 64;
    const int ch = a.col_ch0 + local / nbx, bx = local - (local / nbx) * nbx;
    const int c = bx * 64 + (threadIdx.x & 63), g = threadIdx.x >> 6;
    const int rbeg = ch * a.chunk, rend = min(mv_wg_col_rows(a), rbeg + a.chunk);
    if (rbeg >= rend && a.cnt) return;
    float s = 0.0f;
    if (c < a.col_n)
        for (int row = rbeg + g; row < rend; row += 4) s += a.colX[(size_t)row * a.col_ld + c];
    red[g][threadIdx.x & 63] = s;
    __syncthreads();
    if (g == 0 && c < a.col_n) a.colslab[(size_t)ch * a.col_n + c] = (red[0][threadIdx.x] + red[1][threadIdx.x]) + (red[2][threadIdx.x] + red[3][threadIdx.x]);
}

__global__ __launch_bounds__(MV_THREADS) void k_wgrad_net(WgradNetArgs a) {
    constexpr int LD = 80;
    __shared__ __attribute__((aligned(16))) float Pt[64 * LD];
    __shared__ __attribute__((aligned(16))) float Qt[64 * LD];
    int bid = blockIdx.x;
    if (a.xcd_runs) {
        const int x = bid & 7, i = bid >> 3;
        bid = (((i >> 4) << 3) + x) * 16 + (i & 15);
        if (bid >= a.nblocks) return;
    }
    if (a.colX && bid >= a.col_blk0) { mv_colsum_block(a, bid - a.col_blk0, Pt); return; }
    const int tid = threadIdx.x, lane = tid & 63, w = __builtin_amdgcn_readfirstlane(tid >> 6), r = lane & 15, q = lane >> 4;
    int l = 0;
    while (l + 1 < a.n_layers && bid >= a.L[l + 1].blk0) ++l;
    const WgradLayer& L = a.L[l];
    const int local = bid - L.blk0, nb = L.nbx * L.nby;
    const int chl = local / nb, rem = local - chl * nb, by = rem / L.nbx, bx = rem - by * L.nbx;
    const int ch = L.ch0 + chl;
    const int i0 = bx * 64, o0 = by * 64, No = L.No, Ki = L.Ki;
    const int rbeg = ch * a.chunk, rend = min(mv_wg_rows(a, L), rbeg + a.chunk);
    if (rbeg >= rend && a.cnt) return;
    f32x4 acc[4];
#pragma unroll
    for (int t = 0; t < 4; ++t) acc[t] = f32x4{0.f, 0.f, 0.f, 0.f};
    float bsum = 0.0f;
    const bool do_bias = bx == 0;
    CH_PH_DECL
    const int npairs = L.P2 ? 2 : 1;
    const int nrb = (rend - rbeg + 63) / 64, nst = npairs * nrb;
    const bool fast = ((L.ldp1 & 3) == 0) && ((L.ldq1 & 3) == 0) && ((((size_t)L.P1) & 15) == 0) && ((((size_t)L.Q1) & 15) == 0) && o0 + 64 <= No && i0 + 64 <= Ki &&
                      (!L.P2 || (((L.ldp2 & 3) == 0) && ((L.ldq2 & 3) == 0) && ((((size_t)L.P2) & 15) == 0) && ((((size_t)L.Q2) & 15) == 0))) && nst > 0;
    if (fast) {
        float4 pv[4], qv[4];
        auto issue = [&](int st) {
            const int pair = st >= nrb ? 1 : 0, rb = rbeg + (st - pair * nrb) * 64;
            const float* P = pair ? L.P2 : L.P1;
            const float* Q = pair ? L.Q2 : L.Q1;
            const int ldp = pair ? L.ldp2 : L.ldp1, ldq = pair ? L.ldq2 : L.ldq1;
#pragma unroll
            for (int u = 0; u < 4; ++u) {
                const int idx = u * MV_THREADS + tid, rr = idx >> 4, c4 = (idx & 15) * 4;
                const int row = min(rb + rr, rend - 1);
                pv[u] = *(const float4*)(P + (size_t)row * ldp + o0 + c4);
                qv[u] = *(const float4*)(Q + (size_t)row * ldq + i0 + c4);
            }
        };
        auto store = [&](int st) {
            const int pair = st >= nrb ? 1 : 0, rb = rbeg + (st - pair * nrb) * 64;
#pragma unroll
            for (int u = 0; u < 4; ++u) {
                const int idx = u * MV_THREADS + tid, rr = idx >> 4, c4 = (idx & 15) * 4;
                const bool in = rb + rr < rend;
                *(float4*)(Pt + rr * LD + c4) = in ? pv[u] : make_float4(0.f, 0.f, 0.f, 0.f);
                *(float4*)(Qt + rr * LD + c4) = in ? qv[u] : make_float4(0.f, 0.f, 0.f, 0.f);
            }
        };
        auto compute = [&](int st) {
            if (do_bias && st < nrb && tid < 64) {
                for (int rr = 0; rr < 64; ++rr) bsum += Pt[rr * LD + tid];
            }
            float av[2], bq[2][4];
            const float* pa = Pt + q * LD + 16 * w + r;
            const float* pb = Qt + q * LD + r;
            av[0] = pa[0];
#pragma unroll
            for (int t = 0; t < 4; ++t) bq[0][t] = pb[16 * t];
#pragma unroll
            for (int s = 0; s < 16; ++s) {
                if (s + 1 < 16) {
                    av[(s + 1) & 1] = pa[4 * (s + 1) * LD];
#pragma unroll
                    for (int t = 0; t < 4; ++t) bq[(s + 1) & 1][t] = pb[4 * (s + 1) * LD + 16 * t];
                }
                __builtin_amdgcn_sched_barrier(0);
#pragma unroll
                for (int t = 0; t < 4; ++t) acc[t] = __builtin_amdgcn_mfma_f32_16x16x4f32(av[s & 1], bq[s & 1][t], acc[t], 0, 0, 0);
                __builtin_amdgcn_sched_barrier(0);
            }
        };
        issue(0);
        for (int st = 0; st + 1 < nst; ++st) {
            __syncthreads();
            store(st);
            __syncthreads();
            issue(st + 1);
            compute(st);
        }
        __syncthreads();
        store(nst - 1);
        __syncthreads();
        compute(nst - 1);
    } else
    for (int pair = 0; pair < npairs; ++pair) {
        const float* P = pair ? L.P2 : L.P1;
        const float* Q = pair ? L.Q2 : L.Q1;
        const int ldp = pair ? L.ldp2 : L.ldp1, ldq = pair ? L.ldq2 : L.ldq1;
        for (int rb = rbeg; rb < rend; rb += 64) {
            CH_PH(0)
            __syncthreads();
            CH_PH(1)
            wg_stage(P, ldp, rb, rend, o0, No, Pt, LD, tid);
            wg_stage(Q, ldq, rb, rend, i0, Ki, Qt, LD, tid);
            CH_PH(2)
            __syncthreads();
            CH_PH(3)
            if (do_bias && pair == 0 && tid < 64) {
                for (int rr = 0; rr < 64; ++rr) bsum += Pt[rr * LD + tid];
            }
            CH_PH(4)
#pragma unroll 4
            for (int s = 0; s < 16; ++s) {
                const float av = Pt[(4 * s + q) * LD + 16 * w + r];
#pragma unroll
                for (int t = 0; t < 4; ++t)
                    acc[t] = __builtin_amdgcn_mfma_f32_16x16x4f32(av, Qt[(4 * s + q) * LD + 16 * t + r], acc[t], 0, 0, 0);
            }
        }
    }
    CH_PH(5)
    float* slab = L.slab + (size_t)ch * No * Ki;
#pragma unroll
    for (int t = 0; t < 4; ++t) {
        const int i = i0 + 16 * t + r;
        if (i < Ki) {
#pragma unroll
            for (int e = 0; e < 4; ++e) {
                const int o = o0 + 16 * w + 4 * q + e;
                if (o < No) slab[(size_t)o * Ki + i] = acc[t][e];
            }
        }
    }
    if (do_bias && tid < 64 && o0 + tid < No) L.bslab[(size_t)ch * No + o0 + tid] = bsum;
    CH_PH(6)
    WG_PH_END(a.L[1].blk0 + 1)
}

__global__ void k_reduce_net(WgradNetArgs a) {
    const unsigned total = a.wtotal + a.btotal;
    for (unsigned i = blockIdx.x * blockDim.x + threadIdx.x; i < total; i += gridDim.x * blockDim.x) {
        const bool isb = i >= a.wtotal;
        const unsigned k = isb ? i - a.wtotal : i;
        int l = 0;
        if (isb) { while (l + 1 < a.n_layers && k >= a.L[l + 1].boff) ++l; }
        else { while (l + 1 < a.n_layers && k >= a.L[l + 1].woff) ++l; }
        const WgradLayer& L = a.L[l];
        float v = 0.0f;
        if (isb) {
            const unsigned j = k - L.boff;
            const float* sp = L.bslab + j;
            const int nchb = a.cnt ? (mv_wg_rows(a, L) + a.chunk - 1) / a.chunk : L.nchunks;
            for (int c = 0; c < nchb; ++c) v += sp[(size_t)c * L.No];
            L.db[j] = v;
        } else {
            const unsigned j = k - L.woff;
            const size_t nk = (size_t)L.No * L.Ki;
            const float* sp = L.slab + j;
            const int nch = a.cnt ? (mv_wg_rows(a, L) + a.chunk - 1) / a.chunk : L.nchunks;
            for (int c = 0; c < nch; c += 8) {
                float t[8];
#pragma unroll
                for (int u = 0; u < 8; ++u) t[u] = sp[(size_t)(c + u < nch ? c + u : nch - 1) * nk];
#pragma unroll
                for (int u = 0; u < 8; ++u) if (c + u < nch) v += t[u];
            }
            if (a.colslab && l == a.col_layer && j < (unsigned)a.col_n) {
                const int ncc = a.cnt ? (mv_wg_col_rows(a) + a.chunk - 1) / a.chunk : a.col_nchunks;
                for (int c = 0; c < ncc; ++c) v += a.colslab[(size_t)c * a.col_n + j];
            }
            L.dW[j] = v;
        }
    }
}

__global__ void k_colsum(const float* __restrict__ X, int ld, int M, int n, int chunk, float* __restrict__ part) {
    __shared__ float red[4][64];
    const int c = blockIdx.x * 64 + (threadIdx.x & 63), g = threadIdx.x >> 6, ch = blockIdx.y;
    const int rbeg = ch * chunk, rend = min(M, rbeg + chunk);
    float s = 0.0f;
    if (c < n)
        for (int row = rbeg + g; row < rend; row += 4) s += X[(size_t)row * ld + c];
    red[g][threadIdx.x & 63] = s;
    __syncthreads();
    if (g == 0 && c < n) part[(size_t)ch * n + c] = (red[0][threadIdx.x] + red[1][threadIdx.x]) + (red[2][threadIdx.x] + red[3][threadIdx.x]);
}

template <class NET>
struct ChainArgsT {
    NET net;
    NET netT;
    int S, M, row_ld0;
    const float* dy; int ld_dy;
    const float* Z[MV_MAXL]; const float* U[MV_MAXL];
    const float* w_last_row0;
    const float* ZB2[MV_MAXL];
    float* ZB[MV_MAXL];
    float* H0B;
    const float* VB0;
    float* VB[MV_MAXL];
    float* ZB2o[MV_MAXL];
    const float* H0; const float* G0;
// ... 839 lines not shown
```

mvsdf_amd/csrc/step_driver.hip:

```cpp
#include <hip/hip_runtime.h>
#include <stdint.h>
#include <stdlib.h>
#include <string.h>
#include <new>
#include "capi_util.h"
#include "step_internal.h"
#include <sched.h>
#include <time.h>

namespace {

inline size_t al256(size_t x) { return (x + 255) & ~(size_t)255; }

struct FwdOffsets {
    size_t w[MVSDF_STEP_MAX_LAYERS], wp[MVSDF_STEP_MAX_LAYERS], wpT[MVSDF_STEP_MAX_LAYERS], wp16[MVSDF_STEP_MAX_LAYERS];
    size_t wx3[MVSDF_STEP_MAX_LAYERS], wx3T[MVSDF_STEP_MAX_LAYERS];
    int chain_x3;
    size_t trace_ws, trace_ws_bytes;
    size_t inv, true_rows, true_rank, counts, view_sorted;
    size_t x_eval, y_eval, n_eval, sdf_ctx, rgb_sorted, render_ctx;
};
struct BwdOffsets {
    size_t dy, dn, dy_x, dn_x, din, drgb_sorted, render_ws, wsA, wsX, dx, fbar;
};
// ... 379 lines not shown
    Step* st = (Step*)step;
    if (!st || !counts) return mv_fail(-1, "mvsdf_step_wait_counts: null argument");
    if (!st->counts_pending) return mv_fail(-1, "mvsdf_step_wait_counts: no forward is in flight");
    if (!st->counts_host_dev) {
        ST_HIP(hipEventSynchronize(st->ev_counts));
        for (int i = 0; i < 4; ++i) counts[i] = st->counts_host[i];
        st->counts_pending = false;
        return 0;
    }
    const int rc = step_wait_seq(st, st->counts_seq, counts);
    st->counts_pending = false;
    return rc;
}

long long mvsdf_step_seq(void* step) { return step ? ((Step*)step)->counts_seq : -1; }
size_t mvsdf_step_counts_offset(void* step) { return step ? ((Step*)step)->fo.counts : 0; }
int mvsdf_step_can_defer(void* step) { Step* st = (Step*)step; return (st && st->can_defer) ? 1 : 0; }
int mvsdf_step_saved_offsets(void* step, size_t out[6]) {
    Step* st = (Step*)step;
    if (!st || !out) return mv_fail(-1, "mvsdf_step_saved_offsets: null argument");
    out[0] = st->fo.x_eval; out[1] = st->fo.y_eval; out[2] = st->fo.n_eval; out[3] = st->fo.view_sorted; out[4] = st->fo.render_ctx; out[5] = st->fo.rgb_sorted;
    return 0;
}

int mvsdf_step_wait_counts_seq(void* step, long long seq, long long counts[4]) {
    Step* st = (Step*)step;
    if (!st || !counts) return mv_fail(-1, "mvsdf_step_wait_counts_seq: null argument");
    if (seq <= 0 || seq > st->counts_seq || !st->counts_host) return mv_fail(-1, "mvsdf_step_wait_counts_seq: no such forward");
    if (!st->counts_host_dev) {
        if (seq != st->counts_seq) return mv_fail(-4, "mvsdf_step_wait_counts_seq: the record of that forward was overwritten (read the counts from its forward block)");
        ST_HIP(hipEventSynchronize(st->ev_counts));
        for (int i = 0; i < 4; ++i) counts[i] = st->counts_host[i];
        return 0;
    }
    if (seq + MVSDF_STEP_COUNT_RING <= st->counts_seq) return mv_fail(-4, "mvsdf_step_wait_counts_seq: the record of that forward was overwritten (read the counts from its forward block)");
    const int rc = step_wait_seq(st, seq, counts);
    if (rc == 0 && seq == st->counts_seq) st->counts_pending = false;
    return rc;
}

long long mvsdf_step_done_seq(void* step, long long counts[4]) {
    Step* st = (Step*)step;
    if (!st || !st->counts_host || !st->counts_host_dev) return 0;
    for (long long seq = st->counts_seq; seq > 0 && seq + MVSDF_STEP_COUNT_RING > st->counts_seq; --seq) {
        long long* slot = st->counts_host + 8 * (seq % MVSDF_STEP_COUNT_RING);
        if (__atomic_load_n(&slot[4], __ATOMIC_ACQUIRE) != seq) continue;
        if (counts) {
            for (int i = 0; i < 4; ++i) counts[i] = slot[i];
            if (__atomic_load_n(&slot[4], __ATOMIC_ACQUIRE) != seq) continue;
        }
        return seq;
    }
    return 0;
}

static int step_backward_impl(void* step, const MvsdfStepParams* prm, int N, int n_true, int d_mask, int e_mask, int use_geo, const float* d_diff,
                        const float* d_rgb, const float* d_gth, const float* d_eo, const float* d_si, const void* fwd_, void* bwd_,
                        float* const* dv, float* const* dg, float* const* db, int accumulate, void* stream) {
    Step* st = (Step*)step;
    if (!st || !prm || !fwd_ || !bwd_ || !dv || !dg || !db) return mv_fail(-1, "mvsdf_step_backward: null argument");
    const MvsdfStepDesc& d = st->d;
    const int R = st->R, E = st->E, M = st->M, nl = st->nl, Nout = st->Nout;
    hipStream_t s = (hipStream_t)stream;
    const char* fwd = (const char*)fwd_;
    const long long* cnt = nullptr;
    int n_hint = -1;
    if (N < 0) {
        if (!st->can_defer) return mv_fail(-3, "mvsdf_step_backward: N < 0 (device-side counts) is not available for this step (mvsdf_step_can_defer)");
        cnt = (const long long*)(fwd + st->fo.counts);
        n_hint = (n_true >= 0 && n_true <= R) ? n_true : R;
        N = R; n_true = R;
    }
    if (N < 0 || N > R || n_true < 0 || n_true > N) return mv_fail(-1, "mvsdf_step_backward: bad counts");
    char* bwd = (char*)bwd_;
    const MvsdfStepLayout& L = st->lay;
    const FwdOffsets& fo = st->fo;
    const BwdOffsets& bo = st->bo;
    MvsdfNetDesc sdf, sdfT, rnd, rndT;
    make_descs(*st, prm, fwd, &sdf, &sdfT, &rnd, &rndT);
    const int Mb = E + N;
    float* dflat = (float*)(bwd + L.dflat);
    float* dW_s = dflat + st->seg[0][0]; float* db_s = dflat + st->seg[0][1];
    float* dW_r = dflat + st->seg[1][0]; float* db_r = dflat + st->seg[1][1];
    float* dy = (float*)(bwd + bo.dy); float* dn = (float*)(bwd + bo.dn);
    const float* x_eval = (const float*)(fwd + fo.x_eval); const float* n_eval = (const float*)(fwd + fo.n_eval);
    const float* view_sorted = (const float*)(fwd + fo.view_sorted); const long long* true_rows = (const long long*)(fwd + fo.true_rows);
    const float* ctx = (const float*)(fwd + fo.sdf_ctx);
    const int dv_ = (d.view_spec & 0x100) ? 0 : 3 + 6 * (d.view_spec & 0xff), dnr = (d.view_spec & 0x200) ? 0 : 3;
    const int nrm0 = dnr ? 3 + dv_ : -1, feat0 = 3 + dv_ + dnr;
    if (Mb == 0) {
        ST_HIP(hipMemsetAsync(dflat, 0, L.dflat_floats * 4, s));
    } else {
        const float* din = nullptr;
        const bool with_r = N > 0 && d_rgb;
        if (with_r) {
            float* drgb_sorted = (float*)(bwd + bo.drgb_sorted);
            float* din_w = (float*)(bwd + bo.din);
            int rcb = mv_render_backward_chain(&rnd, &rndT, N, R, d_rgb, (const long long*)(fwd + L.perm), (const float*)(fwd + fo.render_ctx), din_w,
                                               (float*)(bwd + bo.render_ws), cnt, stream);
            if (rcb == -3 && !cnt) {
                hipLaunchKernelGGL(k_step_gather_drgb, dim3((3 * N + 255) / 256), dim3(256), 0, s, d_rgb, (const long long*)(fwd + L.perm), N, drgb_sorted);
                rcb = mv_render_backward_chain(&rnd, &rndT, N, R, drgb_sorted, nullptr, (const float*)(fwd + fo.render_ctx), din_w, (float*)(bwd + bo.render_ws), nullptr, stream);
            }
            if (rcb) return rcb;
            din = din_w;
        } else {
            ST_HIP(hipMemsetAsync(dflat + st->seg[1][0], 0, (st->seg[1][2] - st->seg[1][0]) * 4, s));
        }
        const float* rctx = with_r ? (const float*)(fwd + fo.render_ctx) : nullptr;
        float* rws = with_r ? (float*)(bwd + bo.render_ws) : nullptr;
        float* wsA = (float*)(bwd + bo.wsA);
        bool done = false;
        if (cnt && !(din && N > 0)) return mv_fail(-3, "mvsdf_step_backward: device-side counts need the upstream of rgb_values (the fused route)");
        if (din && N > 0) {
            float* dy_x = (float*)(bwd + bo.dy_x); float* dn_x = (float*)(bwd + bo.dn_x);
            ST_TRY(mv_step_backward_assemble(d.n_eik, d.n_ds, N, Nout, n_true, din, st->K0r, feat0, nrm0, use_geo, (const int*)(fwd + fo.true_rank), d_eo,
                                             d_gth, d_si, d_mask, e_mask, dy, dn, dy_x, dn_x, cnt, stream));
            float* dx = (float*)(bwd + bo.dx);
            int rc = mv_sdf_backward_pair_cnt(&sdf, &sdfT, M, M, Mb, dy, dn, wsA, E, N, dy_x, use_geo ? dn_x : nullptr, (float*)(bwd + bo.wsX), dx, ctx, cnt, n_hint, stream);
            if (rc == 0) {
                float* fbar = (float*)(bwd + bo.fbar);
                if (mv_delta_is_chain() && !cnt) {
                    ST_TRY(mvsdf_step_backward_fbar(d.n_eik, d.n_ds, N, Nout, din, st->K0r, use_geo, d_diff, dx, view_sorted, n_eval, dy, fbar, stream));
                    ST_TRY(mv_sdf_backward_delta(&sdf, &sdfT, M, M, Mb, ctx, wsA, E, N, fbar, stream));
                } else {
                    ST_TRY(mv_sdf_backward_delta_fbar(&sdf, M, M, Mb, ctx, wsA, E, N, Nout, din, st->K0r, use_geo, d_diff, dx, view_sorted, n_eval, dy, fbar, cnt, stream));
                }
                ST_TRY(mv_step_wgrad(&sdf, &rnd, M, M, Mb, dy, ctx, wsA, with_r ? N : 0, R, rctx, rws, dW_s, db_s, dW_r, db_r, cnt, E, stream));
                done = true;
            } else if (rc == -3 && !cnt) {
                ST_TRY(mvsdf_sdf_backward(&sdf, &sdfT, x_eval + 3 * (size_t)E, M, M, E, N, dy_x, use_geo ? dn_x : nullptr, ctx, nullptr, nullptr, dx, wsA, stream));
                float* fbar = (float*)(bwd + bo.fbar);
                ST_TRY(mvsdf_step_backward_fbar(d.n_eik, d.n_ds, N, Nout, din, st->K0r, use_geo, d_diff, dx, view_sorted, n_eval, dy, fbar, stream));
            } else {
                return rc;
            }
        } else {
            ST_TRY(mvsdf_step_backward_inputs(0, d.n_eik, d.n_ds, N, Nout, n_true, din, st->K0r, feat0, nrm0, use_geo, nullptr, nullptr, view_sorted, n_eval,
                                              true_rows, nullptr, nullptr, nullptr, d_mask, e_mask, dy, dn, stream));
            ST_TRY(mvsdf_step_backward_inputs(1, d.n_eik, d.n_ds, N, Nout, n_true, din, st->K0r, feat0, nrm0, use_geo, d_diff, nullptr, view_sorted, n_eval,
                                              true_rows, d_eo, d_gth, d_si, d_mask, e_mask, dy, dn, stream));
        }
        if (!done) {
            ST_TRY(mvsdf_sdf_backward(&sdf, &sdfT, x_eval, M, M, 0, Mb, dy, dn, ctx, dW_s, db_s, nullptr, wsA, stream));
            if (with_r) {
                float* drgb_sorted = (float*)(bwd + bo.drgb_sorted);
                hipLaunchKernelGGL(k_step_gather_drgb, dim3((3 * N + 255) / 256), dim3(256), 0, s, d_rgb, (const long long*)(fwd + L.perm), N, drgb_sorted);
                ST_TRY(mvsdf_render_backward(&rnd, &rndT, N, R, drgb_sorted, rctx, dW_r, db_r, (float*)(bwd + bo.din), rws, stream));
            }
        }
    }
    const float* dWl[MVSDF_STEP_MAX_LAYERS]; const float* dbl[MVSDF_STEP_MAX_LAYERS];
    for (int l = 0; l < nl; ++l) { dWl[l] = dflat + st->woff[l]; dbl[l] = dflat + st->boff[l]; }
    return mvsdf_fold_backward_net(nl, prm->v, prm->g, dWl, dbl, d.N, d.K, dv, dg, db, accumulate ? 1 : 0, stream);
}

int mvsdf_step_backward(void* step, const MvsdfStepParams* prm, int N, int n_true, int d_mask, int e_mask, int use_geo, const float* d_diff,
                        const float* d_rgb, const float* d_gth, const float* d_eo, const float* d_si, const void* fwd_, void* bwd_,
                        float* const* dv, float* const* dg, float* const* db, int accumulate, void* stream) {
    Step* st = (Step*)step;
    const bool timing = st && st->timing;
    if (timing) ST_HIP(hipEventRecord(st->ev_t[6], (hipStream_t)stream));
    const int rc = step_backward_impl(step, prm, N, n_true, d_mask, e_mask, use_geo, d_diff, d_rgb, d_gth, d_eo, d_si, fwd_, bwd_, dv, dg, db, accumulate, stream);
    if (rc) return rc;
    if (timing) { ST_HIP(hipEventRecord(st->ev_t[7], (hipStream_t)stream)); st->timed_bwd = true; }
    return 0;
}

}

extern "C" int mvsdf_abi_struct_sizes(size_t* out) {
    if (!out) return mv_fail(-1, "mvsdf_abi_struct_sizes: null argument");
    out[0] = sizeof(MvsdfNetDesc); out[1] = sizeof(MvsdfTraceParams); out[2] = sizeof(MvsdfStepDesc); out[3] = sizeof(MvsdfStepParams);
    out[4] = sizeof(MvsdfStepInputs); out[5] = sizeof(MvsdfStepLayout); out[6] = sizeof(MvsdfLossArgs); out[7] = sizeof(MvsdfLossLayout);
    return 8;
}
```

mvsdf_amd/csrc/step_internal.h:

```cpp
#pragma once
#include <stdint.h>
#include "../../include/mvsdf_hip.h"

struct FwdGather { const float* eik; const float* on; const float* jit; const float* pts; const long long* perm; int n_eik, n_ds; float* x_out; };

int mv_partition_rays_step(const uint8_t* net_mask, const uint8_t* object_mask, const uint8_t* true_mask, const float* ray_dirs, int R, long long* perm,
                           long long* inv, long long* true_rows, long long* counts, float* view_sorted, int* true_rank, const long long* extra_counts,
                           long long* counts_host, long long counts_seq, float* term_rows, int n_eik, int n_ds, int d_mask, int e_mask,
                           void* stream);
int mv_step_backward_assemble(int n_eik, int n_ds, int N, int Nout, int n_true, const float* din, int din_ld, int din_feat0, int din_nrm0, int use_geo,
                              const int* true_rank, const float* d_eo, const float* d_gth, const float* d_si, int d_mask, int e_mask, float* dy,
                              float* dn, float* dy_x, float* dn_x, const long long* cnt, void* stream);

int mv_sdf_backward_pair_cnt(const MvsdfNetDesc* d, const MvsdfNetDesc* dT, int M, int Mg, int MbA, const float* dyA, const float* dnA, float* wsA,
                             int row0X, int MbX, const float* dyX, const float* dnX, float* wsX, float* dx, const float* ctx, const long long* cnt, int n_hint,
                             void* stream);
int mv_step_can_defer(const MvsdfNetDesc* sdf, const MvsdfNetDesc* sdfT, const MvsdfNetDesc* rnd, const MvsdfNetDesc* rndT);

int mv_sdf_forward_gather(const MvsdfNetDesc* d, const MvsdfNetDesc* dT, const float* x, const void* gather, int M, int Mg, int r_begin, int r_end,
                          float* y, float* nrm, float* ctx, void* stream);
int mv_chain_split_pays(const MvsdfNetDesc* d, int E, int M);

int mv_render_backward_chain(const MvsdfNetDesc* d, const MvsdfNetDesc* dT, int N, int Nctx, const float* drgb, const long long* drgb_rows, const float* ctx,
                             float* din, float* ws, const long long* cnt, void* stream);
int mv_delta_is_chain();
int mv_sdf_backward_delta_fbar(const MvsdfNetDesc* d, int M, int Mg, int Mb, const float* ctx, float* ws, int row0D, int MbD, int Nout, const float* din,
                               int din_ld, int use_geo, const float* d_diff, const float* dx, const float* view_sorted, const float* n_eval, float* dy,
                               float* fbar, const long long* cnt, void* stream);
int mv_sdf_backward_delta(const MvsdfNetDesc* d, const MvsdfNetDesc* dT, int M, int Mg, int Mb, const float* ctx, float* ws, int row0D, int MbD,
                          const float* fbar, void* stream);
int mv_step_wgrad(const MvsdfNetDesc* sd, const MvsdfNetDesc* rd, int M, int Mg, int Mb, const float* dy, const float* ctx, float* wsA, int N, int Nctx,
                  const float* rctx, float* rws, float* dW_s, float* db_s, float* dW_r, float* db_r, const long long* cnt, int cnt_base, void* stream);

int mv_step_prologue(int n_layers, const float* const* v, const float* const* g, const int* N, const int* K, float* const* w, float* const* wp,
                     float* const* wpT, void* const* wp16, const int* nsplit, int wp16_mode, void* const* wx3, void* const* wx3T, const float* uv, const float* pose,
                     const float* intrinsics, int B, int P,
                     float* ray_dirs, float* cam_loc, uint8_t* ones, unsigned long long* counters, const float* stage_src, float* stage_a, int stage_na,
                     float* stage_b, int stage_nb, void* stream);
int mv_chain_x3_enabled();
extern "C" int mv_trace_stage1_prezeroed(const MvsdfNetDesc* desc, const MvsdfTraceParams* tp, const float* cam_loc, const float* ray_dirs, const uint8_t* object_mask,
                              int B, int P, int training, const float* intervals, const float* minsdf_steps, float* points, uint8_t* mask, float* dists,
                              unsigned long long* counters, void* workspace, size_t workspace_bytes, int mt, int rpw, void* stream);
```

mvsdf_amd/ops.py:

```python
import ctypes as C

import torch

from ._lib import NetDesc, TraceParams, check, lib, ptr, stream_of


def _f32(t):
    assert t.dtype == torch.float32 and t.is_cuda, 'expected a float32 CUDA(HIP) tensor'
    return t.contiguous()


class PackedLayer:
    __slots__ = ('w', 'wp', 'wpT', 'bias', 'K', 'N', 'wp16', 'wp_ptr', 'wpT_ptr', 'w_ptr', 'keep', 'wx3', 'wx3T')


class PackedNet:

    def __init__(self, layers, skip_layer, multires):
        self.skip_layers = tuple(sorted(int(s) for s in skip_layer)) if isinstance(skip_layer, (tuple, list)) else ((int(skip_layer),) if skip_layer >= 0 else ())
        self.layers, self.multires = layers, multires
        self.skip_layer = self.skip_layers[0] if self.skip_layers else -1
        self.trace_dtype = 0

    def desc(self, transposed=False):
# ... 87 lines not shown
            w0 = off
            for l in range(lo, hi):
                self.woff[l] = off; off += shapes[l][0] * shapes[l][1]
            b0 = off
            for l in range(lo, hi):
                self.boff[l] = off; off += shapes[l][0]
            self.seg.append((w0, b0, off))
            lo = hi
        self.total = off
        self.poff, self.pToff = [], []
        po = 0
        for (N, K) in shapes:
            self.poff.append(po); po += lib().mvsdf_packed_floats(N, K)
            self.pToff.append(po); po += lib().mvsdf_packed_floats(K, N)
        self.ptotal = po
        self._param_key, self._param_arrays = None, None

    def param_arrays(self, vs, gs, bs):
        key = tuple(p.data_ptr() for p in vs) + tuple(p.data_ptr() for p in bs) + tuple(0 if p is None else p.data_ptr() for p in gs) \
            + tuple(0 if p.grad is None else p.grad.data_ptr() for p in vs) + tuple(0 if p.grad is None else p.grad.data_ptr() for p in bs) \
            + tuple(0 if (p is None or p.grad is None) else p.grad.data_ptr() for p in gs)
        if self._param_key != key:
            g_ok = all(p.grad is not None for p in list(vs) + list(bs)) and all(g is None or g.grad is not None for g in gs)
            self._param_arrays = (_ptr_array([v.detach() for v in vs]), _ptr_array([g.detach() if g is not None else None for g in gs]),
                                  (_ptr_array([v.grad for v in vs]), _ptr_array([g.grad if g is not None else None for g in gs]),
                                   _ptr_array([b.grad for b in bs])) if g_ok else None)
            self._param_key = key
        return self._param_arrays


def fold_pack_net_flat(plan, vs, gs, bs, layers):
    dev = vs[0].device
    flat = torch.empty(plan.total, dtype=torch.float32, device=dev)
    packs = torch.empty(plan.ptotal, dtype=torch.float32, device=dev)
    fb, pb = flat.data_ptr(), packs.data_ptr()
    wps, wpTs, wss = [], [], []
    for l, L in enumerate(layers):
        L.w = L.wp = L.wpT = None
        L.w_ptr, L.wp_ptr, L.wpT_ptr = fb + 4 * plan.woff[l], pb + 4 * plan.poff[l], pb + 4 * plan.pToff[l]
        wss.append(L.w_ptr); wps.append(L.wp_ptr); wpTs.append(L.wpT_ptr)
    pv, pg, _ = plan.param_arrays(vs, gs, bs)
    check(lib().mvsdf_fold_pack_net(plan.n, pv, pg, plan.N, plan.K, _int_ptr_array(wss), _int_ptr_array(wps), _int_ptr_array(wpTs),
                                    stream_of(vs[0])), 'mvsdf_fold_pack_net')
    return flat, packs


def fold_backward_net_flat(plan, vs, gs, bs, dflat, sink):
    base = dflat.data_ptr()
    dW = _int_ptr_array([base + 4 * o for o in plan.woff])
    db = _int_ptr_array([base + 4 * o for o in plan.boff])
    pv, pg, grads = plan.param_arrays(vs, gs, bs)
    if sink and grads is not None:
        check(lib().mvsdf_fold_backward_net(plan.n, pv, pg, dW, db, plan.N, plan.K, grads[0], grads[1], grads[2], 1, stream_of(dflat)),
              'mvsdf_fold_backward_net')
        return None
    dvs = [torch.empty_like(v) for v in vs]
    dgs = [torch.empty_like(g) if g is not None else None for g in gs]
    check(lib().mvsdf_fold_backward_net(plan.n, pv, pg, dW, None, plan.N, plan.K, _ptr_array(dvs), _ptr_array(dgs), None, 0, stream_of(dflat)),
          'mvsdf_fold_backward_net')
    dbs = [dflat[o:o + s[0]] for o, s in zip(plan.boff, plan.shapes)]
    return dvs, dgs, dbs


def fold_backward_net(vs, gs, dWs, dbs=None, sinks=None):
    vs = [_f32(v) for v in vs]
    gs = [_f32(g).reshape(-1) if g is not None else None for g in gs]
    dWs = [_f32(d) for d in dWs]
    n = len(vs)
    N = (C.c_int * n)(*[v.shape[0] for v in vs])
    K = (C.c_int * n)(*[v.shape[1] for v in vs])
    if sinks is not None:
        tv, tg, tb = sinks
        for t in list(tv) + list(tg) + list(tb):
            assert t is None or (t.is_cuda and t.dtype == torch.float32 and t.is_contiguous())
        dbs = [_f32(d) for d in dbs]
        check(lib().mvsdf_fold_backward_net(n, _ptr_array(vs), _ptr_array(gs), _ptr_array(dWs), _ptr_array(dbs), N, K, _ptr_array(tv),
                                            _ptr_array(tg), _ptr_array(tb), 1, stream_of(vs[0])), 'mvsdf_fold_backward_net')
        return None
    dvs = [torch.empty_like(v) for v in vs]
    dgs = [torch.empty_like(g) if g is not None else None for g in gs]
    check(lib().mvsdf_fold_backward_net(n, _ptr_array(vs), _ptr_array(gs), _ptr_array(dWs), None, N, K, _ptr_array(dvs), _ptr_array(dgs),
                                        None, 0, stream_of(vs[0])), 'mvsdf_fold_backward_net')
    return dvs, [g.reshape(-1, 1) if g is not None else None for g in dgs]


CHAIN_X3 = True


def pack_x3_chain(net):
    n = len(net.layers)
    dev = net.layers[0].bias.device
    N = (C.c_int * n)(*[L.N for L in net.layers])
    K = (C.c_int * n)(*[L.K for L in net.layers])
    ws = _int_ptr_array([L.w.data_ptr() if L.w is not None else L.w_ptr for L in net.layers])
    for L in net.layers:
        L.wx3 = torch.empty(3 * lib().mvsdf_packed_bf16_bytes(L.N, L.K, 0), dtype=torch.uint8, device=dev)
        L.wx3T = torch.empty(3 * lib().mvsdf_packed_bf16_bytes(L.K, L.N, 0), dtype=torch.uint8, device=dev)
    s = stream_of(net.layers[0].bias)
    check(lib().mvsdf_pack_bf16x3_net(n, ws, N, K, _ptr_array([L.wx3 for L in net.layers]), s), 'mvsdf_pack_bf16x3_net')
    check(lib().mvsdf_pack_bf16x3t_net(n, ws, N, K, _ptr_array([L.wx3T for L in net.layers]), s), 'mvsdf_pack_bf16x3t_net')
    net.__dict__.pop('_d', None)
    net.__dict__.pop('_dT', None)
    return net


def pack_net(vs, gs, biases, skip_layer, multires, want_t=True, x3=None):
    layers = []
    for v, g, b in zip(vs, gs, biases):
        L = PackedLayer()
        L.w, L.wp, L.wpT = fold_pack(v, g, want_t)
        L.bias = _f32(b)
        L.N, L.K = v.shape
        L.wp16 = None
        L.wx3 = L.wx3T = None
        layers.append(L)
    net = PackedNet(layers, skip_layer, multires)
    if (CHAIN_X3 if x3 is None else x3) and want_t:
        maybe_pack_x3_chain(net, force=x3)
    return net


def maybe_pack_x3_chain(net, force=None):
    if (CHAIN_X3 if force is None else force) and len(net.layers) >= 2 and net.layers[0].K == 3 + 6 * max(net.multires, 0):
        pack_x3_chain(net)
    return net


TRACE_DTYPES = {'f32': 0, 'bf16w': 2, 'bf16x2': 3, 'bf16x3': 4, 'f32x3': 5}


def pack_trace_net(net, dtype):
    if dtype == 'f32':
        return net
    return pack_bf16_net(net, weights_only=(dtype == 'bf16w'), terms={'bf16x2': 2, 'bf16x3': 3, 'f32x3': 3}.get(dtype, 0), weight_terms=3 if dtype == 'f32x3' else 1)


def pack_bf16_net(net, weights_only=False, terms=0, weight_terms=1):
    n = len(net.layers)
    if terms:
        assert terms in (2, 3) and not weights_only and weight_terms in (1, 3) and (weight_terms == 1 or terms == 3)
        dev = net.layers[0].bias.device
        for L in net.layers:
            L.wp16 = torch.empty(weight_terms * lib().mvsdf_packed_bf16_bytes(L.N, L.K, 0), dtype=torch.uint8, device=dev)
        N = (C.c_int * n)(*[L.N for L in net.layers])
        K = (C.c_int * n)(*[L.K for L in net.layers])
        fn = lib().mvsdf_pack_bf16x3_net if weight_terms == 3 else lib().mvsdf_pack_bf16s_net
        check(fn(n, _int_ptr_array([L.w.data_ptr() if L.w is not None else L.w_ptr for L in net.layers]), N, K,
                 _ptr_array([L.wp16 for L in net.layers]), stream_of(net.layers[0].bias)), 'mvsdf_pack_bf16s_net / mvsdf_pack_bf16x3_net')
        net.trace_dtype = 5 if weight_terms == 3 else 1 + terms
        net.__dict__.pop('_d', None)
        return net
    if weights_only:
        dev = net.layers[0].bias.device
        for L in net.layers:
            L.wp16 = torch.empty(lib().mvsdf_packed_floats(L.N, L.K), dtype=torch.float32, device=dev)
        N = (C.c_int * n)(*[L.N for L in net.layers])
        K = (C.c_int * n)(*[L.K for L in net.layers])
        check(lib().mvsdf_pack_bf16w_net(n, _int_ptr_array([L.w.data_ptr() if L.w is not None else L.w_ptr for L in net.layers]), N, K,
                                         _ptr_array([L.wp16 for L in net.layers]), stream_of(net.layers[0].bias)), 'mvsdf_pack_bf16w_net')
        net.trace_dtype = 2
        net.__dict__.pop('_d', None)
        return net
    raise ValueError("pack_bf16_net: give weights_only=True ('bf16w') or terms=2 / 3 ('bf16x2' / 'bf16x3'; with weight_terms=3: 'f32x3') -- the engine that rounded the "
                     "hidden activations to bf16 too (trace_dtype 1) was removed in round 5")


# ... 433 lines not shown
```

Baseline: 1.383 million.

## Fuse weight-gradient slab reduction into weight-norm fold backward kernel

Adds a kernel that reduces the per-chunk weight-gradient slabs (plus column sums and bias slabs) and applies the weight-norm fold backward for every layer in a single launch. In the training step, the separate slab-reduction launch and the later fold-backward launch are replaced by this one. The goal is to avoid writing the reduced dW to memory and reading it back, and to drop a launch. The change also adds a chunk-major block ordering for wgrad and a vectorised wgrad block path. The cost is more complex per-row code, with the slab reads now happening inside the fold kernel.

```diff
diff --git a/include/mvsdf_hip.h b/include/mvsdf_hip.h
--- a/include/mvsdf_hip.h
+++ b/include/mvsdf_hip.h
@@ -63,6 +63,10 @@
 int mvsdf_fold_backward_net(int n_layers, const float* const* v, const float* const* g, const float* const* dW, const float* const* db,
                             const int* N, const int* K, float* const* dv, float* const* dg, float* const* dbias, int accumulate,
                             void* stream);
+int mvsdf_fold_backward_slabs_net(int n_layers, const float* const* v, const float* const* g, const float* const* slab, const float* const* bslab,
+                                  const int* nchunks, const int* mbase, int chunk, const long long* cnt, const float* colslab, int col_layer, int col_n,
+                                  int col_nchunks, int col_mbase, const int* N, const int* K, float* const* dW, float* const* db, float* const* dv,
+                                  float* const* dg, float* const* dbias, int accumulate, void* stream);
 int mvsdf_fold_backward(const float* v, const float* g, const float* dW, int N, int K, float* dv, float* dg, void* stream);
 
 size_t mvsdf_packed_bf16_bytes(int N, int K, int nsplit);
@@ -116,6 +120,12 @@
                             int row0X, int MbX, const float* dyX, const float* dnX, float* wsX, float* dx, const float* ctx, void* stream);
 int mvsdf_sdf_backward_finish(const MvsdfNetDesc* net, const MvsdfNetDesc* netT, int M, int Mg, int Mb, const float* dy, const float* ctx, float* ws,
                               int row0D, int MbD, const float* fbar, float* dW_cat, float* db_cat, void* stream);
+
+size_t mvsdf_wgrad_layer_ws_floats(int M, int No, int Ki);
+int mvsdf_wgrad_layer(const float* P, int ldp, const float* Q, int ldq, int M, int No, int Ki, float* ws, float* dW, float* db, void* stream);
+int mvsdf_wgrad_reduce_net(int n_layers, const float* const* slab, const float* const* bslab, const int* nchunks, const int* mbase, int chunk,
+                           const long long* cnt, const float* colslab, int col_layer, int col_n, int col_nchunks, int col_mbase, const int* N,
+                           const int* K, float* const* dW, float* const* db, void* stream);
 
 size_t mvsdf_render_ctx_floats(const MvsdfNetDesc* net, int N);
 size_t mvsdf_render_bwd_ws_floats(const MvsdfNetDesc* net, int N);
diff --git a/mvsdf_amd/_lib.py b/mvsdf_amd/_lib.py
--- a/mvsdf_amd/_lib.py
+++ b/mvsdf_amd/_lib.py
@@ -128,6 +128,11 @@
         L.mvsdf_batch_args_bytes.restype = sz
         L.mvsdf_batch_args_bytes.argtypes = []
         L.mvsdf_batch_gather.argtypes = [vp, vp]
+        L.mvsdf_wgrad_layer_ws_floats.restype = sz
+        L.mvsdf_wgrad_layer_ws_floats.argtypes = [C.c_int] * 3
+        L.mvsdf_wgrad_layer.argtypes = [vp, C.c_int, vp, C.c_int] + [C.c_int] * 3 + [vp] * 4
+        L.mvsdf_wgrad_reduce_net.argtypes = [C.c_int] + [vp] * 4 + [C.c_int, vp, vp] + [C.c_int] * 4 + [vp] * 5
+        L.mvsdf_fold_backward_slabs_net.argtypes = [C.c_int] + [vp] * 6 + [C.c_int, vp, vp] + [C.c_int] * 4 + [vp] * 7 + [C.c_int, vp]
         for name in EXPORTS:
             getattr(L, name)
         _lib = L
@@ -140,6 +145,7 @@
     'mvsdf_tracegen_state_bytes', 'mvsdf_tracegen_init', 'mvsdf_tracegen_step', 'mvsdf_tracegen_finish', 'mvsdf_tracegen_rows', 'mvsdf_tracegen_reduce',
     'mvsdf_tracegen_secant',
     'mvsdf_sdf_ctx_floats', 'mvsdf_sdf_forward', 'mvsdf_sdf_bwd_ws_floats', 'mvsdf_sdf_backward', 'mvsdf_sdf_backward_pair', 'mvsdf_sdf_backward_finish',
+    'mvsdf_wgrad_layer_ws_floats', 'mvsdf_wgrad_layer', 'mvsdf_wgrad_reduce_net', 'mvsdf_fold_backward_slabs_net',
     'mvsdf_feat_corr', 'mvsdf_depth_carve', 'mvsdf_loss_terms', 'mvsdf_loss_prep', 'mvsdf_loss_scale', 'mvsdf_adam_ws_floats', 'mvsdf_adam_step', 'mvsdf_adam_step_scaled', 'mvsdf_adam_step_fused',
     'mvsdf_partition_rays', 'mvsdf_step_outputs', 'mvsdf_step_backward_inputs', 'mvsdf_step_backward_fbar', 'mvsdf_dsurf_select', 'mvsdf_dsurf_points',
     'mvsdf_render_ctx_floats', 'mvsdf_render_bwd_ws_floats', 'mvsdf_render_forward', 'mvsdf_render_backward',
diff --git a/mvsdf_amd/csrc/basic.hip b/mvsdf_amd/csrc/basic.hip
--- a/mvsdf_amd/csrc/basic.hip
+++ b/mvsdf_amd/csrc/basic.hip
@@ -4,6 +4,7 @@
 #include "trace_params.h"
 #include "capi_util.h"
 #include "det_math_pk.h"
+#include "step_internal.h"
 
 __global__ __launch_bounds__(256) void k_fold(const float* __restrict__ v, const float* __restrict__ g, int N, int K, float* __restrict__ w) {
     const int j = blockIdx.x * 4 + (threadIdx.x >> 6), lane = threadIdx.x & 63;
@@ -144,6 +145,162 @@
         a.dg[l][j] = acc ? a.dg[l][j] + dgj : dgj;
         if (a.db[l]) a.dbias[l][j] = acc ? a.dbias[l][j] + a.db[l][j] : a.db[l][j];
     }
+}
+
+__device__ __forceinline__ float mv_fs_add_chunks(float v, const float* __restrict__ p, size_t stride, int n) {
+    for (int c = 0; c < n; c += 8) {
+        float t[8];
+#pragma unroll
+        for (int u = 0; u < 8; ++u) t[u] = p[(size_t)(c + u < n ? c + u : n - 1) * stride];
+#pragma unroll
+        for (int u = 0; u < 8; ++u) if (c + u < n) v += t[u];
+    }
+    return v;
+}
+template <int NC>
+__device__ __forceinline__ void mv_fs_row(const MvFoldSlabArgs& a, const MvFoldSlabLayer& L, int l, int j, int lane, int nch, int ncc, float* dd) {
+    const int K = L.K;
+    const size_t nk = (size_t)L.N * K, j0 = (size_t)j * K;
+    if (!L.slab) {
+#pragma unroll
+        for (int c = 0; c < NC; ++c) { const int k = 64 * c + lane; const float y = L.dW[j0 + (k < K ? k : K - 1)]; dd[c] = k < K ? y : 0.0f; }
+        return;
+    }
+    const float* sp = L.slab + j0;
+#pragma unroll
+    for (int c = 0; c < NC; ++c) dd[c] = 0.0f;
+#pragma unroll
+    for (int cb = 0; cb < NC; cb += 4) {
+        for (int c0 = 0; c0 < nch; c0 += 8) {
+            float t[4][8];
+#pragma unroll
+            for (int c = cb; c < cb + 4 && c < NC; ++c) {
+                const int k = 64 * c + lane, kc = k < K ? k : K - 1;
+#pragma unroll
+                for (int u = 0; u < 8; ++u) t[c - cb][u] = sp[(size_t)(c0 + u < nch ? c0 + u : nch - 1) * nk + kc];
+            }
+#pragma unroll
+            for (int c = cb; c < cb + 4 && c < NC; ++c) {
+#pragma unroll
+                for (int u = 0; u < 8; ++u) if (c0 + u < nch) dd[c] += t[c - cb][u];
+            }
+        }
+    }
+    const bool col = a.colslab && l == a.col_layer && j0 < (size_t)a.col_n;
+#pragma unroll
+    for (int c = 0; c < NC; ++c) {
+        const int k = 64 * c + lane;
+        if (col && k < K && j0 + k < (size_t)a.col_n) dd[c] = mv_fs_add_chunks(dd[c], a.colslab + j0 + k, (size_t)a.col_n, ncc);
+        if (k < K) L.dW[j0 + k] = dd[c]; else dd[c] = 0.0f;
+    }
+}
+template <int NC>
+__device__ __forceinline__ void mv_fs_fold_row(const MvFoldSlabArgs& a, const MvFoldSlabLayer& L, int l, int j, int lane, int nch, int ncc, float dbj) {
+    const int K = L.K;
+    const float* vr = L.v + (size_t)j * K;
+    float* dvr = L.dv + (size_t)j * K;
+    const bool acc = a.accumulate != 0;
+    float vv[NC], dd[NC], old[NC];
+    const float gj = L.g[j];
+#pragma unroll
+    for (int c = 0; c < NC; ++c) {
+        const int k = 64 * c + lane, kc = k < K ? k : K - 1;
+        const float x = vr[kc], z = acc ? dvr[kc] : 0.0f;
+        vv[c] = k < K ? x : 0.0f; old[c] = z;
+    }
+    mv_fs_row<NC>(a, L, l, j, lane, nch, ncc, dd);
+    float ss = 0.f, dot = 0.f;
+#pragma unroll
+    for (int c = 0; c < NC; ++c) if (64 * c < K) { ss = fmaf(vv[c], vv[c], ss); dot = fmaf(dd[c], vv[c], dot); }
+    for (int o = 32; o > 0; o >>= 1) { ss += __shfl_xor(ss, o); dot += __shfl_xor(dot, o); }
+    const float inv = 1.0f / sqrtf(ss);
+    const float dgj = dot * inv, s = gj * inv;
+#pragma unroll
+    for (int c = 0; c < NC; ++c) {
+        const int k = 64 * c + lane;
+        if (k < K) { const float t = s * (dd[c] - dgj * vv[c] * inv); dvr[k] = acc ? old[c] + t : t; }
+    }
+    if (lane == 0) {
+        L.dg[j] = acc ? L.dg[j] + dgj : dgj;
+        if (L.dbias) L.dbias[j] = acc ? L.dbias[j] + dbj : dbj;
+    }
+}
+__global__ __launch_bounds__(256) void k_fold_bwd_slabs(MvFoldSlabArgs a) {
+    const int l = blockIdx.y;
+    const MvFoldSlabLayer& L = a.L[l];
+    const int N = L.N, K = L.K;
+    const int j = __builtin_amdgcn_readfirstlane(blockIdx.x * 4 + (threadIdx.x >> 6)), lane = threadIdx.x & 63;
+    if (j >= N) return;
+    const int nch = a.cnt ? (L.mbase + (int)a.cnt[0] + a.chunk - 1) / a.chunk : L.nchunks;
+    const int ncc = a.cnt ? (a.col_mbase + (int)a.cnt[0] + a.chunk - 1) / a.chunk : a.col_nchunks;
+    float dbj = 0.0f;
+    if (L.slab) {
+        for (int c0 = 0; c0 < nch; c0 += 64) {
+            const float mine = c0 + lane < nch ? L.bslab[(size_t)(c0 + lane) * N + j] : 0.0f;
+            const int n = min(64, nch - c0);
+            for (int i = 0; i < n; ++i) dbj += __int_as_float(__builtin_amdgcn_readlane(__float_as_int(mine), i));
+        }
+        if (lane == 0) L.db[j] = dbj;
+    } else if (L.dbias) dbj = L.db[j];
+    const bool acc = a.accumulate != 0;
+    if (L.g && K <= 64 * 9) {
+        switch ((K + 63) >> 6) {
+            case 1: mv_fs_fold_row<1>(a, L, l, j, lane, nch, ncc, dbj); break;
+            case 2: mv_fs_fold_row<2>(a, L, l, j, lane, nch, ncc, dbj); break;
+            case 3: mv_fs_fold_row<3>(a, L, l, j, lane, nch, ncc, dbj); break;
+            case 4: mv_fs_fold_row<4>(a, L, l, j, lane, nch, ncc, dbj); break;
+            case 5: mv_fs_fold_row<5>(a, L, l, j, lane, nch, ncc, dbj); break;
+            case 6: mv_fs_fold_row<6>(a, L, l, j, lane, nch, ncc, dbj); break;
+            case 7: mv_fs_fold_row<7>(a, L, l, j, lane, nch, ncc, dbj); break;
+            case 8: mv_fs_fold_row<8>(a, L, l, j, lane, nch, ncc, dbj); break;
+            default: mv_fs_fold_row<9>(a, L, l, j, lane, nch, ncc, dbj); break;
+        }
+        return;
+    }
+    float* dr = L.dW + (size_t)j * K;
+    if (L.slab) {
+        const size_t nk = (size_t)N * K, j0 = (size_t)j * K;
+        const bool col = a.colslab && l == a.col_layer && j0 < (size_t)a.col_n;
+        for (int k = lane; k < K; k += 64) {
+            float x = mv_fs_add_chunks(0.0f, L.slab + j0 + k, nk, nch);
+            if (col && j0 + k < (size_t)a.col_n) x = mv_fs_add_chunks(x, a.colslab + j0 + k, (size_t)a.col_n, ncc);
+            dr[k] = x;
+        }
+    }
+    const float* vr = L.v + (size_t)j * K;
+    float* dvr = L.dv + (size_t)j * K;
+    if (!L.g) {
+        for (int k = lane; k < K; k += 64) dvr[k] = acc ? dvr[k] + dr[k] : dr[k];
+        if (lane == 0 && L.dbias) L.dbias[j] = acc ? L.dbias[j] + dbj : dbj;
+        return;
+    }
+    float ss = 0.f, dot = 0.f;
+    for (int k = lane; k < K; k += 64) { ss = fmaf(vr[k], vr[k], ss); dot = fmaf(dr[k], vr[k], dot); }
+    for (int o = 32; o > 0; o >>= 1) { ss += __shfl_xor(ss, o); dot += __shfl_xor(dot, o); }
+    const float inv = 1.0f / sqrtf(ss);
+    const float dgj = dot * inv, s = L.g[j] * inv;
+    for (int k = lane; k < K; k += 64) {
+        const float t = s * (dr[k] - dgj * vr[k] * inv);
+        dvr[k] = acc ? dvr[k] + t : t;
+    }
+    if (lane == 0) {
+        L.dg[j] = acc ? L.dg[j] + dgj : dgj;
+        if (L.dbias) L.dbias[j] = acc ? L.dbias[j] + dbj : dbj;
+    }
+}
+
+int mv_fold_backward_slabs(const MvFoldSlabArgs* a, void* stream) {
+    if (!a || a->n_layers < 1 || a->n_layers > MV_FS_MAXL || a->chunk <= 0) return mv_fail(-1, "mv_fold_backward_slabs: bad arguments");
+    int maxN = 0;
+    for (int l = 0; l < a->n_layers; ++l) {
+        const MvFoldSlabLayer& L = a->L[l];
+        if (L.N <= 0 || L.K <= 0 || !L.v || !L.dv || !L.dW || (L.g && !L.dg) || (L.slab && (!L.bslab || !L.db || L.nchunks < 1)) || (!L.slab && L.dbias && !L.db))
+            return mv_fail(-1, "mv_fold_backward_slabs: bad layer arguments");
+        if (L.N > maxN) maxN = L.N;
+    }
+    if (a->colslab && (a->col_layer < 0 || a->col_layer >= a->n_layers || a->col_n <= 0 || a->col_nchunks < 1)) return mv_fail(-1, "mv_fold_backward_slabs: bad column sums");
+    hipLaunchKernelGGL(k_fold_bwd_slabs, dim3((maxN + 3) / 4, a->n_layers), dim3(256), 0, (hipStream_t)stream, *a);
+    return mv_check(hipGetLastError(), "mv_fold_backward_slabs");
 }
 
 __global__ void k_fold_bwd(const float* __restrict__ v, const float* __restrict__ g, const float* __restrict__ dW, int N, int K,
@@ -417,6 +574,25 @@
     }
     hipLaunchKernelGGL(k_fold_bwd_net, dim3((maxN + 3) / 4, n_layers), dim3(256), 0, (hipStream_t)stream, a);
     return mv_check(hipGetLastError(), "mvsdf_fold_backward_net");
+}
+
+int mvsdf_fold_backward_slabs_net(int n_layers, const float* const* v, const float* const* g, const float* const* slab, const float* const* bslab,
+                                  const int* nchunks, const int* mbase, int chunk, const long long* cnt, const float* colslab, int col_layer, int col_n,
+                                  int col_nchunks, int col_mbase, const int* N, const int* K, float* const* dW, float* const* db, float* const* dv,
+                                  float* const* dg, float* const* dbias, int accumulate, void* stream) {
+    if (n_layers < 1 || n_layers > MV_FS_MAXL || !v || !g || !slab || !bslab || !nchunks || !N || !K || !dW || !db || !dv || !dg)
+        return mv_fail(-1, "mvsdf_fold_backward_slabs_net: bad arguments");
+    MvFoldSlabArgs a;
+    memset(&a, 0, sizeof(a));
+    a.n_layers = n_layers; a.chunk = chunk; a.accumulate = accumulate; a.cnt = cnt;
+    a.colslab = colslab; a.col_layer = col_layer; a.col_n = col_n; a.col_nchunks = col_nchunks; a.col_mbase = col_mbase;
+    for (int l = 0; l < n_layers; ++l) {
+        MvFoldSlabLayer& L = a.L[l];
+        L.slab = slab[l]; L.bslab = bslab[l]; L.dW = dW[l]; L.db = db[l]; L.v = v[l]; L.g = g[l]; L.dv = dv[l]; L.dg = dg[l];
+        L.dbias = dbias ? dbias[l] : nullptr;
+        L.N = N[l]; L.K = K[l]; L.nchunks = nchunks[l]; L.mbase = mbase ? mbase[l] : 0;
+    }
+    return mv_fold_backward_slabs(&a, stream);
 }
 
 int mvsdf_fold_backward(const float* v, const float* g, const float* dW, int N, int K, float* dv, float* dg, void* stream) {
diff --git a/mvsdf_amd/csrc/diff_mlp.hip b/mvsdf_amd/csrc/diff_mlp.hip
--- a/mvsdf_amd/csrc/diff_mlp.hip
+++ b/mvsdf_amd/csrc/diff_mlp.hip
@@ -208,6 +208,20 @@
     for (int l = 0; l < a.n_layers; ++l) {
         WgradLayer& L = a.L[l];
         L.blk0 = blk; blk += L.nbx * L.nby * L.nch;
+    }
+    static int order_env = -2;
+    if (order_env == -2) { const char* e = mv_dev_env("MVSDF_WG_ORDER"); order_env = (e && *e) ? atoi(e) : -1; }
+    a.cm_n = 0;
+    if (order_env != 0) {
+        int c0 = 0, b0 = 0;
+        while (a.cm_n < MV_WG_MAXL) {
+            int nb = 0, next = 0;
+            for (int l = 0; l < a.n_layers; ++l)
+                if (a.L[l].nch > c0) { nb += a.L[l].nbx * a.L[l].nby; next = (!next || a.L[l].nch < next) ? a.L[l].nch : next; }
+            if (!nb) break;
+            a.cm_c0[a.cm_n] = c0; a.cm_blk0[a.cm_n] = b0; a.cm_nb[a.cm_n] = nb; ++a.cm_n;
+            b0 += nb * (next - c0); c0 = next;
+        }
     }
     if (a.colX) { a.col_blk0 = blk; blk += ((a.col_n + 63) / 64) * a.col_nch; }
     static int xcd_env = -2;
@@ -846,6 +860,44 @@
     wgrad_colsum(wa, ws + bl.VB[nl - 1], Ki, Mb, Ki, nl - 1, bl.nchunks, ws + bl.slabB);
     MV_TRY(launch_wgrad_net(wa, s));
     return mv_check(hipGetLastError(), "mvsdf_sdf_backward_finish");
+}
+
+size_t mvsdf_wgrad_layer_ws_floats(int M, int No, int Ki) {
+    if (M <= 0 || No <= 0 || Ki <= 0) return 0;
+    return (size_t)((M + MV_WG_CHUNK - 1) / MV_WG_CHUNK) * ((size_t)No * Ki + No);
+}
+
+int mvsdf_wgrad_layer(const float* P, int ldp, const float* Q, int ldq, int M, int No, int Ki, float* ws, float* dW, float* db, void* stream) {
+    if (!P || !Q || !ws || !dW || !db || M <= 0 || No <= 0 || Ki <= 0 || ldp < No || ldq < Ki) return mv_fail(-1, "mvsdf_wgrad_layer: bad arguments");
+    WgradNetArgs wa;
+    memset(&wa, 0, sizeof(wa));
+    const int nchunks = (M + MV_WG_CHUNK - 1) / MV_WG_CHUNK;
+    wa.n_layers = 1; wa.chunk = MV_WG_CHUNK;
+    WgradLayer& L = wa.L[0];
+    L.P1 = P; L.ldp1 = ldp; L.Q1 = Q; L.ldq1 = ldq; L.No = No; L.Ki = Ki;
+    wgrad_net_layers(wa, 0, 1, M, nchunks, ws, ws + (size_t)nchunks * No * Ki, dW, db);
+    MV_TRY(launch_wgrad_net(wa, (hipStream_t)stream));
+    return mv_check(hipGetLastError(), "mvsdf_wgrad_layer");
+}
+
+int mvsdf_wgrad_reduce_net(int n_layers, const float* const* slab, const float* const* bslab, const int* nchunks, const int* mbase, int chunk,
+                           const long long* cnt, const float* colslab, int col_layer, int col_n, int col_nchunks, int col_mbase, const int* N,
+                           const int* K, float* const* dW, float* const* db, void* stream) {
+    if (n_layers < 1 || n_layers > MV_WG_MAXL || !slab || !bslab || !nchunks || !N || !K || !dW || !db || chunk <= 0 ||
+        (colslab && (col_layer < 0 || col_layer >= n_layers || col_n <= 0 || col_nchunks < 1)))
+        return mv_fail(-1, "mvsdf_wgrad_reduce_net: bad arguments");
+    WgradNetArgs wa;
+    memset(&wa, 0, sizeof(wa));
+    wa.n_layers = n_layers; wa.chunk = chunk; wa.cnt = cnt;
+    wa.colslab = const_cast<float*>(colslab); wa.col_layer = col_layer; wa.col_n = col_n; wa.col_nchunks = col_nchunks; wa.col_mbase = col_mbase;
+    for (int l = 0; l < n_layers; ++l) {
+        WgradLayer& L = wa.L[l];
+        if (!slab[l] || !bslab[l] || !dW[l] || !db[l] || N[l] <= 0 || K[l] <= 0 || nchunks[l] < 1) return mv_fail(-1, "mvsdf_wgrad_reduce_net: bad layer arguments");
+        L.slab = const_cast<float*>(slab[l]); L.bslab = const_cast<float*>(bslab[l]); L.dW = dW[l]; L.db = db[l];
+        L.No = N[l]; L.Ki = K[l]; L.nchunks = nchunks[l]; L.mbase = mbase ? mbase[l] : 0;
+    }
+    MV_TRY(wgrad_reduce(wa, (hipStream_t)stream));
+    return mv_check(hipGetLastError(), "mvsdf_wgrad_reduce_net");
 }
 
 }
@@ -1077,8 +1129,10 @@
     return mv_check(hipGetLastError(), "mv_sdf_backward_delta_fbar");
 }
 
+static_assert(MV_FS_MAXL == MV_WG_MAXL, "MvFoldSlabArgs holds the layers of one k_wgrad_net launch");
 int mv_step_wgrad(const MvsdfNetDesc* sd, const MvsdfNetDesc* rd, int M, int Mg, int Mb, const float* dy, const float* ctx, float* wsA, int N, int Nctx,
-                  const float* rctx, float* rws, float* dW_s, float* db_s, float* dW_r, float* db_r, const long long* cnt, int cnt_base, void* stream) {
+                  const float* rctx, float* rws, float* dW_s, float* db_s, float* dW_r, float* db_r, const long long* cnt, int cnt_base, MvFoldSlabArgs* fs,
+                  void* stream) {
     MvNet net, rnet;
     int rc = mv_make_net(sd, &net);
     if (rc) return rc;
@@ -1109,6 +1163,17 @@
         for (int l = 0; l < nl; ++l) wa.L[l].mbase = cnt_base;
         for (int l = nl; l < nl + nr; ++l) wa.L[l].mbase = 0;
     }
+    if (fs) {
+        MV_TRY(wgrad_launch(wa, (hipStream_t)stream));
+        fs->n_layers = wa.n_layers; fs->chunk = wa.chunk; fs->cnt = wa.cnt;
+        fs->colslab = wa.colslab; fs->col_layer = wa.col_layer; fs->col_n = wa.col_n; fs->col_nchunks = wa.col_nchunks; fs->col_mbase = wa.col_mbase;
+        for (int l = 0; l < wa.n_layers; ++l) {
+            const WgradLayer& L = wa.L[l];
+            MvFoldSlabLayer& F = fs->L[l];
+            F.slab = L.slab; F.bslab = L.bslab; F.dW = L.dW; F.db = L.db; F.N = L.No; F.K = L.Ki; F.nchunks = L.nchunks; F.mbase = L.mbase;
+        }
+        return mv_check(hipGetLastError(), "mv_step_wgrad");
+    }
     MV_TRY(launch_wgrad_net(wa, (hipStream_t)stream));
     return mv_check(hipGetLastError(), "mv_step_wgrad");
 }
diff --git a/mvsdf_amd/csrc/layer_kernels.h b/mvsdf_amd/csrc/layer_kernels.h
--- a/mvsdf_amd/csrc/layer_kernels.h
+++ b/mvsdf_amd/csrc/layer_kernels.h
@@ -173,43 +173,6 @@
     }
 }
 
-__device__ __forceinline__ void wg_stage(const float* __restrict__ src, int ld, int row_lo, int row_hi, int c0, int ncols, float* __restrict__ dst,
-                                         int LD, int tid) {
-    const bool vec = ((ld & 3) == 0) && ((c0 & 3) == 0) && ((((size_t)src) & 15) == 0);
-    if (vec) {
-        float4 v[4];
-#pragma unroll
-        for (int u = 0; u < 4; ++u) {
-            const int idx = u * MV_THREADS + tid, rr = idx >> 4, c4 = (idx & 15) * 4, row = row_lo + rr;
-            v[u] = make_float4(0.f, 0.f, 0.f, 0.f);
-            if (row < row_hi) {
-                if (c0 + c4 + 3 < ncols) v[u] = *(const float4*)(src + (size_t)row * ld + c0 + c4);
-                else {
-                    float t[4] = {0.f, 0.f, 0.f, 0.f};
-                    for (int e = 0; e < 4; ++e) if (c0 + c4 + e < ncols) t[e] = src[(size_t)row * ld + c0 + c4 + e];
-                    v[u] = make_float4(t[0], t[1], t[2], t[3]);
-                }
-            }
-        }
-#pragma unroll
-        for (int u = 0; u < 4; ++u) {
-            const int idx = u * MV_THREADS + tid, rr = idx >> 4, c4 = (idx & 15) * 4;
-            *(float4*)(dst + rr * LD + c4) = v[u];
-        }
-    } else {
-        float v[16];
-#pragma unroll
-        for (int u = 0; u < 16; ++u) {
-            const int idx = u * MV_THREADS + tid, rr = idx >> 6, c = idx & 63, row = row_lo + rr;
-            v[u] = (row < row_hi && c0 + c < ncols) ? src[(size_t)row * ld + c0 + c] : 0.0f;
-        }
-#pragma unroll
-        for (int u = 0; u < 16; ++u) {
-            const int idx = u * MV_THREADS + tid, rr = idx >> 6, c = idx & 63;
-            dst[rr * LD + c] = v[u];
-        }
-    }
-}
 
 #ifdef MV_CHAIN_PROBE
 __device__ unsigned long long g_chain_ph[16][16];
@@ -247,6 +210,7 @@
     unsigned wtotal, btotal;
     const long long* cnt; int col_mbase;
     int xcd_runs, nblocks;
+    int cm_n, cm_c0[MV_WG_MAXL], cm_blk0[MV_WG_MAXL], cm_nb[MV_WG_MAXL];
 };
 
 __device__ __forceinline__ int mv_wg_rows(const WgradNetArgs& a, const WgradLayer& L) { return a.cnt ? L.mbase + (int)a.cnt[0] : L.M; }
@@ -267,7 +231,102 @@
     if (g == 0 && c < a.col_n) a.colslab[(size_t)ch * a.col_n + c] = (red[0][threadIdx.x] + red[1][threadIdx.x]) + (red[2][threadIdx.x] + red[3][threadIdx.x]);
 }
 
-__global__ __launch_bounds__(MV_THREADS) void k_wgrad_net(WgradNetArgs a) {
+template <bool VEC>
+__device__ __forceinline__ void mv_wgrad_block(const WgradLayer& L, int rbeg, int rend, int o0, int i0, bool do_bias, float* __restrict__ Pt, float* __restrict__ Qt,
+                                               f32x4 (&acc)[4], float& bsum) {
+    constexpr int LD = 80;
+    const int tid = threadIdx.x, lane = tid & 63, w = __builtin_amdgcn_readfirstlane(tid >> 6), r = lane & 15, q = lane >> 4;
+    const int No = L.No, Ki = L.Ki;
+    const int nrb = (rend - rbeg + 63) / 64, nst = (L.P2 ? 2 : 1) * nrb;
+    float4 pv[4], qv[4];
+    float pf[16], qf[16];
+    auto issue = [&](int st) {
+        const int pair = st >= nrb ? 1 : 0, rb = rbeg + (st - pair * nrb) * 64;
+        const float* P = pair ? L.P2 : L.P1;
+        const float* Q = pair ? L.Q2 : L.Q1;
+        const int ldp = pair ? L.ldp2 : L.ldp1, ldq = pair ? L.ldq2 : L.ldq1;
+        if constexpr (VEC) {
+#pragma unroll
+            for (int u = 0; u < 4; ++u) {
+                const int idx = u * MV_THREADS + tid, rr = idx >> 4, c4 = (idx & 15) * 4;
+                const int row = min(rb + rr, rend - 1);
+                pv[u] = *(const float4*)(P + (size_t)row * ldp + o0 + c4);
+                qv[u] = *(const float4*)(Q + (size_t)row * ldq + i0 + c4);
+            }
+        } else {
+            const float* Pb = P + (size_t)rb * ldp;
+            const float* Qb = Q + (size_t)rb * ldq;
+            const unsigned c = tid & 63, rl = (unsigned)(min(rb + 64, rend) - 1 - rb);
+            const unsigned cp = min(o0 + (int)c, No - 1), cq = min(i0 + (int)c, Ki - 1);
+            const unsigned p0 = (tid >> 6) * (unsigned)ldp + cp, pmax = rl * (unsigned)ldp + cp;
+            const unsigned q0 = (tid >> 6) * (unsigned)ldq + cq, qmax = rl * (unsigned)ldq + cq;
+#pragma unroll
+            for (int u = 0; u < 16; ++u) {
+                pf[u] = Pb[min(p0 + 4u * u * (unsigned)ldp, pmax)];
+                qf[u] = Qb[min(q0 + 4u * u * (unsigned)ldq, qmax)];
+            }
+        }
+    };
+    auto store = [&](int st) {
+        const int pair = st >= nrb ? 1 : 0, rb = rbeg + (st - pair * nrb) * 64;
+        if constexpr (VEC) {
+#pragma unroll
+            for (int u = 0; u < 4; ++u) {
+                const int idx = u * MV_THREADS + tid, rr = idx >> 4, c4 = (idx & 15) * 4;
+                const bool in = rb + rr < rend;
+                *(float4*)(Pt + rr * LD + c4) = in ? pv[u] : make_float4(0.f, 0.f, 0.f, 0.f);
+                *(float4*)(Qt + rr * LD + c4) = in ? qv[u] : make_float4(0.f, 0.f, 0.f, 0.f);
+            }
+        } else {
+            const int c = tid & 63;
+            const bool inp = o0 + c < No, inq = i0 + c < Ki;
+#pragma unroll
+            for (int u = 0; u < 16; ++u) {
+                const int rr = 4 * u + (tid >> 6);
+                const bool in = rb + rr < rend;
+                Pt[rr * LD + c] = (in && inp) ? pf[u] : 0.0f;
+                Qt[rr * LD + c] = (in && inq) ? qf[u] : 0.0f;
+            }
+        }
+    };
+    auto compute = [&](int st) {
+        if (do_bias && st < nrb && tid < 64) {
+            for (int rr = 0; rr < 64; ++rr) bsum += Pt[rr * LD + tid];
+        }
+        float av[2], bq[2][4];
+        const float* pa = Pt + q * LD + 16 * w + r;
+        const float* pb = Qt + q * LD + r;
+        av[0] = pa[0];
+#pragma unroll
+        for (int t = 0; t < 4; ++t) bq[0][t] = pb[16 * t];
+#pragma unroll
+        for (int s = 0; s < 16; ++s) {
+            if (s + 1 < 16) {
+                av[(s + 1) & 1] = pa[4 * (s + 1) * LD];
+#pragma unroll
+                for (int t = 0; t < 4; ++t) bq[(s + 1) & 1][t] = pb[4 * (s + 1) * LD + 16 * t];
+            }
+            __builtin_amdgcn_sched_barrier(0);
+#pragma unroll
+            for (int t = 0; t < 4; ++t) acc[t] = __builtin_amdgcn_mfma_f32_16x16x4f32(av[s & 1], bq[s & 1][t], acc[t], 0, 0, 0);
+            __builtin_amdgcn_sched_barrier(0);
+        }
+    };
+    issue(0);
+    for (int st = 0; st + 1 < nst; ++st) {
+        __syncthreads();
+        store(st);
+        __syncthreads();
+        issue(st + 1);
+        compute(st);
+    }
+    __syncthreads();
+    store(nst - 1);
+    __syncthreads();
+    compute(nst - 1);
+}
+
+__global__ __launch_bounds__(MV_THREADS, 4) void k_wgrad_net(WgradNetArgs a) {
     constexpr int LD = 80;
     __shared__ __attribute__((aligned(16))) float Pt[64 * LD];
     __shared__ __attribute__((aligned(16))) float Qt[64 * LD];
@@ -279,11 +338,25 @@
     }
     if (a.colX && bid >= a.col_blk0) { mv_colsum_block(a, bid - a.col_blk0, Pt); return; }
     const int tid = threadIdx.x, lane = tid & 63, w = __builtin_amdgcn_readfirstlane(tid >> 6), r = lane & 15, q = lane >> 4;
-    int l = 0;
-    while (l + 1 < a.n_layers && bid >= a.L[l + 1].blk0) ++l;
+    int l = 0, chl, rem;
+    if (a.cm_n) {
+        int k = 0;
+        while (k + 1 < a.cm_n && bid >= a.cm_blk0[k + 1]) ++k;
+        const int rel = bid - a.cm_blk0[k], cs = rel / a.cm_nb[k];
+        chl = a.cm_c0[k] + cs; rem = rel - cs * a.cm_nb[k];
+        for (;; ++l) {
+            if (a.L[l].nch <= chl) continue;
+            const int nbl = a.L[l].nbx * a.L[l].nby;
+            if (rem < nbl) break;
+            rem -= nbl;
+        }
+    } else {
+        while (l + 1 < a.n_layers && bid >= a.L[l + 1].blk0) ++l;
+        const int local = bid - a.L[l].blk0, nb = a.L[l].nbx * a.L[l].nby;
+        chl = local / nb; rem = local - chl * nb;
+    }
     const WgradLayer& L = a.L[l];
-    const int local = bid - L.blk0, nb = L.nbx * L.nby;
-    const int chl = local / nb, rem = local - chl * nb, by = rem / L.nbx, bx = rem - by * L.nbx;
+    const int by = rem / L.nbx, bx = rem - by * L.nbx;
     const int ch = L.ch0 + chl;
     const int i0 = bx * 64, o0 = by * 64, No = L.No, Ki = L.Ki;
     const int rbeg = ch * a.chunk, rend = min(mv_wg_rows(a, L), rbeg + a.chunk);
@@ -294,96 +367,11 @@
     float bsum = 0.0f;
     const bool do_bias = bx == 0;
     CH_PH_DECL
-    const int npairs = L.P2 ? 2 : 1;
-    const int nrb = (rend - rbeg + 63) / 64, nst = npairs * nrb;
-    const bool fast = ((L.ldp1 & 3) == 0) && ((L.ldq1 & 3) == 0) && ((((size_t)L.P1) & 15) == 0) && ((((size_t)L.Q1) & 15) == 0) && o0 + 64 <= No && i0 + 64 <= Ki &&
-                      (!L.P2 || (((L.ldp2 & 3) == 0) && ((L.ldq2 & 3) == 0) && ((((size_t)L.P2) & 15) == 0) && ((((size_t)L.Q2) & 15) == 0))) && nst > 0;
-    if (fast) {
-        float4 pv[4], qv[4];
-        auto issue = [&](int st) {
-            const int pair = st >= nrb ? 1 : 0, rb = rbeg + (st - pair * nrb) * 64;
-            const float* P = pair ? L.P2 : L.P1;
-            const float* Q = pair ? L.Q2 : L.Q1;
-            const int ldp = pair ? L.ldp2 : L.ldp1, ldq = pair ? L.ldq2 : L.ldq1;
-#pragma unroll
-            for (int u = 0; u < 4; ++u) {
-                const int idx = u * MV_THREADS + tid, rr = idx >> 4, c4 = (idx & 15) * 4;
-                const int row = min(rb + rr, rend - 1);
-                pv[u] = *(const float4*)(P + (size_t)row * ldp + o0 + c4);
-                qv[u] = *(const float4*)(Q + (size_t)row * ldq + i0 + c4);
-            }
-        };
-        auto store = [&](int st) {
-            const int pair = st >= nrb ? 1 : 0, rb = rbeg + (st - pair * nrb) * 64;
-#pragma unroll
-            for (int u = 0; u < 4; ++u) {
-                const int idx = u * MV_THREADS + tid, rr = idx >> 4, c4 = (idx & 15) * 4;
-                const bool in = rb + rr < rend;
-                *(float4*)(Pt + rr * LD + c4) = in ? pv[u] : make_float4(0.f, 0.f, 0.f, 0.f);
-                *(float4*)(Qt + rr * LD + c4) = in ? qv[u] : make_float4(0.f, 0.f, 0.f, 0.f);
-            }
-        };
-        auto compute = [&](int st) {
-            if (do_bias && st < nrb && tid < 64) {
-                for (int rr = 0; rr < 64; ++rr) bsum += Pt[rr * LD + tid];
-            }
-            float av[2], bq[2][4];
-            const float* pa = Pt + q * LD + 16 * w + r;
-            const float* pb = Qt + q * LD + r;
-            av[0] = pa[0];
-#pragma unroll
-            for (int t = 0; t < 4; ++t) bq[0][t] = pb[16 * t];
-#pragma unroll
-            for (int s = 0; s < 16; ++s) {
-                if (s + 1 < 16) {
-                    av[(s + 1) & 1] = pa[4 * (s + 1) * LD];
-#pragma unroll
-                    for (int t = 0; t < 4; ++t) bq[(s + 1) & 1][t] = pb[4 * (s + 1) * LD + 16 * t];
-                }
-                __builtin_amdgcn_sched_barrier(0);
-#pragma unroll
-                for (int t = 0; t < 4; ++t) acc[t] = __builtin_amdgcn_mfma_f32_16x16x4f32(av[s & 1], bq[s & 1][t], acc[t], 0, 0, 0);
-                __builtin_amdgcn_sched_barrier(0);
-            }
-        };
-        issue(0);
-        for (int st = 0; st + 1 < nst; ++st) {
-            __syncthreads();
-            store(st);
-            __syncthreads();
-            issue(st + 1);
-            compute(st);
-        }
-        __syncthreads();
-        store(nst - 1);
-        __syncthreads();
-        compute(nst - 1);
-    } else
-    for (int pair = 0; pair < npairs; ++pair) {
-        const float* P = pair ? L.P2 : L.P1;
-        const float* Q = pair ? L.Q2 : L.Q1;
-        const int ldp = pair ? L.ldp2 : L.ldp1, ldq = pair ? L.ldq2 : L.ldq1;
-        for (int rb = rbeg; rb < rend; rb += 64) {
-            CH_PH(0)
-            __syncthreads();
-            CH_PH(1)
-            wg_stage(P, ldp, rb, rend, o0, No, Pt, LD, tid);
-            wg_stage(Q, ldq, rb, rend, i0, Ki, Qt, LD, tid);
-            CH_PH(2)
-            __syncthreads();
-            CH_PH(3)
-            if (do_bias && pair == 0 && tid < 64) {
-                for (int rr = 0; rr < 64; ++rr) bsum += Pt[rr * LD + tid];
-            }
-            CH_PH(4)
-#pragma unroll 4
-            for (int s = 0; s < 16; ++s) {
-                const float av = Pt[(4 * s + q) * LD + 16 * w + r];
-#pragma unroll
-                for (int t = 0; t < 4; ++t)
-                    acc[t] = __builtin_amdgcn_mfma_f32_16x16x4f32(av, Qt[(4 * s + q) * LD + 16 * t + r], acc[t], 0, 0, 0);
-            }
-        }
+    const bool vec = ((L.ldp1 & 3) == 0) && ((L.ldq1 & 3) == 0) && ((((size_t)L.P1) & 15) == 0) && ((((size_t)L.Q1) & 15) == 0) && o0 + 64 <= No && i0 + 64 <= Ki &&
+                     (!L.P2 || (((L.ldp2 & 3) == 0) && ((L.ldq2 & 3) == 0) && ((((size_t)L.P2) & 15) == 0) && ((((size_t)L.Q2) & 15) == 0)));
+    if (rbeg < rend) {
+        if (vec) mv_wgrad_block<true>(L, rbeg, rend, o0, i0, do_bias, Pt, Qt, acc, bsum);
+        else mv_wgrad_block<false>(L, rbeg, rend, o0, i0, do_bias, Pt, Qt, acc, bsum);
     }
     CH_PH(5)
     float* slab = L.slab + (size_t)ch * No * Ki;
diff --git a/mvsdf_amd/csrc/step_driver.hip b/mvsdf_amd/csrc/step_driver.hip
--- a/mvsdf_amd/csrc/step_driver.hip
+++ b/mvsdf_amd/csrc/step_driver.hip
@@ -485,6 +485,9 @@
     float* dflat = (float*)(bwd + L.dflat);
     float* dW_s = dflat + st->seg[0][0]; float* db_s = dflat + st->seg[0][1];
     float* dW_r = dflat + st->seg[1][0]; float* db_r = dflat + st->seg[1][1];
+    MvFoldSlabArgs fs;
+    memset(&fs, 0, sizeof(fs));
+    bool fused_fold = false;
     float* dy = (float*)(bwd + bo.dy); float* dn = (float*)(bwd + bo.dn);
     const float* x_eval = (const float*)(fwd + fo.x_eval); const float* n_eval = (const float*)(fwd + fo.n_eval);
     const float* view_sorted = (const float*)(fwd + fo.view_sorted); const long long* true_rows = (const long long*)(fwd + fo.true_rows);
@@ -529,7 +532,8 @@
                 } else {
                     ST_TRY(mv_sdf_backward_delta_fbar(&sdf, M, M, Mb, ctx, wsA, E, N, Nout, din, st->K0r, use_geo, d_diff, dx, view_sorted, n_eval, dy, fbar, cnt, stream));
                 }
-                ST_TRY(mv_step_wgrad(&sdf, &rnd, M, M, Mb, dy, ctx, wsA, with_r ? N : 0, R, rctx, rws, dW_s, db_s, dW_r, db_r, cnt, E, stream));
+                fused_fold = nl <= MV_FS_MAXL;
+                ST_TRY(mv_step_wgrad(&sdf, &rnd, M, M, Mb, dy, ctx, wsA, with_r ? N : 0, R, rctx, rws, dW_s, db_s, dW_r, db_r, cnt, E, fused_fold ? &fs : nullptr, stream));
                 done = true;
             } else if (rc == -3 && !cnt) {
                 ST_TRY(mvsdf_sdf_backward(&sdf, &sdfT, x_eval + 3 * (size_t)E, M, M, E, N, dy_x, use_geo ? dn_x : nullptr, ctx, nullptr, nullptr, dx, wsA, stream));
@@ -553,6 +557,16 @@
             }
         }
     }
+    if (fused_fold) {
+        for (int l = 0; l < nl; ++l) {
+            MvFoldSlabLayer& F = fs.L[l];
+            if (l >= fs.n_layers) { F.slab = F.bslab = nullptr; F.N = d.N[l]; F.K = d.K[l]; F.dW = dflat + st->woff[l]; F.db = dflat + st->boff[l]; }
+            if (F.dW != dflat + st->woff[l] || F.db != dflat + st->boff[l] || F.N != d.N[l] || F.K != d.K[l]) return mv_fail(-1, "mvsdf_step_backward: weight-gradient slabs and the flat gradient block disagree");
+            F.v = prm->v[l]; F.g = prm->g[l]; F.dv = dv[l]; F.dg = dg[l]; F.dbias = db[l];
+        }
+        fs.n_layers = nl; fs.accumulate = accumulate ? 1 : 0;
+        return mv_fold_backward_slabs(&fs, stream);
+    }
     const float* dWl[MVSDF_STEP_MAX_LAYERS]; const float* dbl[MVSDF_STEP_MAX_LAYERS];
     for (int l = 0; l < nl; ++l) { dWl[l] = dflat + st->woff[l]; dbl[l] = dflat + st->boff[l]; }
     return mvsdf_fold_backward_net(nl, prm->v, prm->g, dWl, dbl, d.N, d.K, dv, dg, db, accumulate ? 1 : 0, stream);
diff --git a/mvsdf_amd/csrc/step_internal.h b/mvsdf_amd/csrc/step_internal.h
--- a/mvsdf_amd/csrc/step_internal.h
+++ b/mvsdf_amd/csrc/step_internal.h
@@ -29,8 +29,23 @@
                                float* fbar, const long long* cnt, void* stream);
 int mv_sdf_backward_delta(const MvsdfNetDesc* d, const MvsdfNetDesc* dT, int M, int Mg, int Mb, const float* ctx, float* ws, int row0D, int MbD,
                           const float* fbar, void* stream);
+#define MV_FS_MAXL 16
+struct MvFoldSlabLayer {
+    const float* slab; const float* bslab;
+    float* dW; float* db;
+    const float* v; const float* g; float* dv; float* dg; float* dbias;
+    int N, K, nchunks, mbase;
+};
+struct MvFoldSlabArgs {
+    int n_layers, chunk, accumulate;
+    const long long* cnt;
+    const float* colslab; int col_layer, col_n, col_nchunks, col_mbase;
+    MvFoldSlabLayer L[MV_FS_MAXL];
+};
+int mv_fold_backward_slabs(const MvFoldSlabArgs* a, void* stream);
 int mv_step_wgrad(const MvsdfNetDesc* sd, const MvsdfNetDesc* rd, int M, int Mg, int Mb, const float* dy, const float* ctx, float* wsA, int N, int Nctx,
-                  const float* rctx, float* rws, float* dW_s, float* db_s, float* dW_r, float* db_r, const long long* cnt, int cnt_base, void* stream);
+                  const float* rctx, float* rws, float* dW_s, float* db_s, float* dW_r, float* db_r, const long long* cnt, int cnt_base, MvFoldSlabArgs* fs,
+                  void* stream);
 
 int mv_step_prologue(int n_layers, const float* const* v, const float* const* g, const int* N, const int* K, float* const* w, float* const* wp,
                      float* const* wpT, void* const* wp16, const int* nsplit, int wp16_mode, void* const* wx3, void* const* wx3T, const float* uv, const float* pose,
diff --git a/mvsdf_amd/ops.py b/mvsdf_amd/ops.py
--- a/mvsdf_amd/ops.py
+++ b/mvsdf_amd/ops.py
@@ -193,6 +193,54 @@
     check(lib().mvsdf_fold_backward_net(n, _ptr_array(vs), _ptr_array(gs), _ptr_array(dWs), None, N, K, _ptr_array(dvs), _ptr_array(dgs),
                                         None, 0, stream_of(vs[0])), 'mvsdf_fold_backward_net')
     return dvs, [g.reshape(-1, 1) if g is not None else None for g in dgs]
+
+
+def wgrad_layer(P, Q):
+    for t in (P, Q):
+        assert t.dtype == torch.float32 and t.is_cuda and t.dim() == 2 and t.stride(1) == 1 and t.stride(0) >= t.shape[1]
+    M, No = P.shape
+    Ki = Q.shape[1]
+    assert Q.shape[0] == M
+    ws = torch.empty(lib().mvsdf_wgrad_layer_ws_floats(M, No, Ki), dtype=torch.float32, device=P.device)
+    dW = torch.empty(No, Ki, dtype=torch.float32, device=P.device)
+    db = torch.empty(No, dtype=torch.float32, device=P.device)
+    check(lib().mvsdf_wgrad_layer(C.c_void_p(P.data_ptr()), P.stride(0), C.c_void_p(Q.data_ptr()), Q.stride(0), M, No, Ki, ptr(ws), ptr(dW), ptr(db),
+                                  stream_of(P)), 'mvsdf_wgrad_layer')
+    return dW, db
+
+
+def _slab_args(slabs, bslabs, chunk, cnt, colslab, col_layer, mbase, col_mbase):
+    n = len(slabs)
+    for s, b in zip(slabs, bslabs):
+        assert s.dtype == torch.float32 and s.is_cuda and s.is_contiguous() and s.dim() == 3 and b.is_contiguous() and b.shape == s.shape[:2]
+    ints = lambda xs: (C.c_int * n)(*xs)
+    return (_ptr_array(slabs), _ptr_array(bslabs), ints([s.shape[0] for s in slabs]), ints(mbase if mbase is not None else [0] * n), chunk, ptr(cnt), ptr(colslab),
+            col_layer, colslab.shape[1] if colslab is not None else 0, colslab.shape[0] if colslab is not None else 0, col_mbase,
+            ints([s.shape[1] for s in slabs]), ints([s.shape[2] for s in slabs]))
+
+
+def wgrad_reduce_net(slabs, bslabs, chunk=256, cnt=None, colslab=None, col_layer=0, mbase=None, col_mbase=0):
+    dWs = [torch.empty_like(s[0]) for s in slabs]
+    dbs = [torch.empty_like(b[0]) for b in bslabs]
+    a = _slab_args(slabs, bslabs, chunk, cnt, colslab, col_layer, mbase, col_mbase)
+    check(lib().mvsdf_wgrad_reduce_net(len(slabs), *a, _ptr_array(dWs), _ptr_array(dbs), stream_of(slabs[0])), 'mvsdf_wgrad_reduce_net')
+    return dWs, dbs
+
+
+def fold_backward_slabs_net(vs, gs, slabs, bslabs, chunk=256, cnt=None, colslab=None, col_layer=0, mbase=None, col_mbase=0, sinks=None):
+    vs = [_f32(v) for v in vs]
+    gs = [_f32(g).reshape(-1) if g is not None else None for g in gs]
+    dWs = [torch.empty_like(s[0]) for s in slabs]
+    dbs = [torch.empty_like(b[0]) for b in bslabs]
+    a = _slab_args(slabs, bslabs, chunk, cnt, colslab, col_layer, mbase, col_mbase)
+    if sinks is not None:
+        dvs, dgs, tb = sinks
+    else:
+        dvs, dgs, tb = [torch.empty_like(v) for v in vs], [torch.empty_like(g) if g is not None else None for g in gs], None
+    check(lib().mvsdf_fold_backward_slabs_net(len(vs), _ptr_array(vs), _ptr_array(gs), *a, _ptr_array(dWs), _ptr_array(dbs), _ptr_array(dvs), _ptr_array(dgs),
+                                              _ptr_array(tb) if tb is not None else None, 1 if sinks is not None else 0, stream_of(vs[0])),
+          'mvsdf_fold_backward_slabs_net')
+    return dWs, dbs, dvs, dgs
 
 
 CHAIN_X3 = True
```

Result: faster. 1.404 million (median of 6 runs) (+1.5%).
